# tesseract-robotics/trajopt

Measured on NVIDIA H100. Metric: converged trajectories/sec (7-DOF x 30 wp, batch 1024), higher is better.
Workload: dtype f64

## Files before the change

trajopt_b200/csrc/device_types.cuh:

```cuda
#pragma once
#include <cstdint>

namespace tb200 {

constexpr int kMaxDof = 16;
constexpr int kMaxSeg = 40;
constexpr int kMaxSpheres = 32;
constexpr int kMaxSteps = 64;

struct DevSegment {
  int parent, joint_type, q_index, pad;
  double R[9];
  double p[3];
  double axis[3];
};
struct DevSphere {
  int segment, pad;
  double c[3];
  double r;
};

enum ObjKind {
  OBJ_JOINT_EQ_COST = 0,
  OBJ_JOINT_INEQ_COST = 1,
  OBJ_JOINT_EQ_CNT = 2,
  OBJ_JOINT_INEQ_CNT = 3,
  OBJ_CART_POSE = 4,
  OBJ_COLL = 5,
  OBJ_CART_VEL = 6,
  OBJ_COLL_CAST = 7
};
struct DevObj {
  int kind;
  int is_cnt;
  int order;
  int first;
  int n_steps;
  int term;
  int src_off;
  int n_rows;
  int link;
  int target_slot;
  int pad0;
  int pad1;
  double coeff, margin, buffer;
  double lvs;
};
struct DevJointTerm {
  double coeffs[kMaxDof], targets[kMaxDof], upper[kMaxDof], lower[kMaxDof];
};
struct DevCartTerm {
  double src_R[9], src_p[3];
  double tgt[7];
  int idx[6];
  double coeff[6];
  int n_idx, pad;
};

enum RowInt { RI_BASE = 0, RI_CNT, RI_STRIDE, RI_AUX, RI_OBJ, RI_PAD, RI_NINTS };
enum AuxKind { AUX_NONE = 0, AUX_HINGE = 1, AUX_ABS = 2 };

struct QpSettings {
  double rho, sigma, alpha, eps_abs, eps_rel, eps_prim_inf, eps_dual_inf, delta, adaptive_rho_tolerance;
  int max_iter, scaling, check_termination, adaptive_rho, adaptive_rho_interval, polishing, polish_refine_iter,
      warm_starting, early_polish_every, early_polish_from;
};
struct SqpParams {
  double improve_ratio_threshold, min_trust_box_size, min_approx_improve, min_approx_improve_frac;
  double trust_shrink_ratio, trust_expand_ratio, cnt_tolerance, max_merit_coeff_increases;
  double merit_coeff_increase_ratio, initial_merit_error_coeff, trust_box_size;
  int max_iter, max_qp_solver_failures, inflate_constraints_individually, pad;
};

struct DevProblem {
  int B, T, D, N, HB;
  int S, L, O, obstacles_per_traj;
  int n_costs, n_cnts, n_cart_rows, cart_stride, n_coll_cand, coll_stride;
  int n_cart_targets, n_fixed, max_rows, row_stride, coll_words;
  int n_sparse_lists, n_band;
  int band_offs[32];
  const DevSegment* segs;
  const DevSphere* spheres;
  const double* lower;
  const double* upper;
  const DevObj* cost_objs;
  const DevObj* cnt_objs;
  const DevJointTerm* joint_terms;
  const DevCartTerm* cart_terms;
  const int* fixed_vars;
  const double* Pband;
  const double* qlin;
  const double* init_traj;
  const double* cart_targets;
  const double* obstacles;
  double* x;
  double* new_x;
  double* trust;
  double* merit_coeffs;
  double* cost_vals;
  double* cnt_viols;
  double* new_cost_vals;
  double* new_cnt_viols;
  double* model_cost_vals;
  double* model_cnt_viols;
  int* status;
  int* sqp_iter;
  int* merit_round;
  int* qp_failures;
  int* qp_status;
  int* cur_buf;
  int* n_qp_solves;
  int* n_func_evals;
  int* n_admm_iters;
  int* active_count;
  double* cart_err;
  double* cart_jac;
  double* coll_rows;
  unsigned long long* coll_mask;
  int n_coll_objs, pad2;
  double* rows;
  int* row_ints;
  int* lists;
  size_t list_stride;
  double* ws_x;
  double* ws_yb;
  double* scratch;
  double* soa;
  size_t soa_stride;
  double* factor_g;
  int* lvs_overflow;
  int* qp_done;
  int* ws_meta;
  double* ws_rho;
  double* trace;
  int* trace_len;
  int trace_cap, pad3;
  double* dbg;
  int* sched_state;
  unsigned long long* sched_timers;
  QpSettings qp;
  SqpParams sqp;
};

}
```

trajopt_b200/csrc/kernels.h:

```cpp
#pragma once
#include "device_types.cuh"

namespace tb200 {
struct EvalExtra;
struct SolveCtl;
using SolveKernelFn = void (*)(DevProblem, EvalExtra, SolveCtl);
using EvalKernelFn = void (*)(DevProblem, EvalExtra, int, const double*);
SolveKernelFn solve_kernel_for(int D, bool pair_rows);
EvalKernelFn eval_kernel_for(int D);
int eval_debug_prof(unsigned long long* out, int reset);
int qp_debug_prof(unsigned long long* out, int reset);
}
```

trajopt_b200/csrc/qp_cta_kernel.cuh:

```cuda
#pragma once
#include "device_types.cuh"
#include "joint_terms.cuh"

namespace tb200 {

#ifdef TB200_PROFILE
static __device__ unsigned long long g_prof[16];
#define PROF_T0() const long long prof_t0_ = clock64()
#define PROF_ADD(slot) do { if (q.tid == 0) atomicAdd(&g_prof[slot], (unsigned long long)(clock64() - prof_t0_)); } while (0)
#else
#define PROF_T0()
#define PROF_ADD(slot)
#endif
#if defined(TB200_PROFILE) && defined(TB200_PROFILE_CHECK)
#define PROF_CHK_T0() long long pc_ = clock64()
#define PROF_CHK(slot) do { const long long n_ = clock64(); if (q.tid == 0) atomicAdd(&g_prof[slot], (unsigned long long)(n_ - pc_)); pc_ = n_; } while (0)
#else
#define PROF_CHK_T0()
#define PROF_CHK(slot)
#endif

constexpr int kQpThreads = 256;
constexpr int kQpThreadsC = 256;
constexpr double kOsqpInf = 1e30;
constexpr double kMinScaling = 1e-4, kMaxScaling = 1e4;
constexpr double kVerifyTol = 1e-9;
constexpr int kVerifyRounds = 3;
constexpr double kRhoMin = 1e-6, kRhoMax = 1e6, kRhoTol = 1e-4, kRhoEqOverIneq = 1e3;
enum { QPS_UNSOLVED = 0, QPS_SOLVED = 1, QPS_SOLVED_INACC = 2, QPS_PINF = 3, QPS_PINF_INACC = 4, QPS_DINF = 5,
       QPS_DINF_INACC = 6, QPS_MAXITER = 7, QPS_NONCVX = 8 };

__device__ __forceinline__ double limit_scaling(double v) {
  v = v < kMinScaling ? 1.0 : v;
  return v > kMaxScaling ? kMaxScaling : v;
}

struct QpSmem {
  int SA, SLM, SU, beta, x, zb, yb, v1, w, qs, lbs, ubs, Dz, v2, Pb, tmp, red, colptr, colent, rints, rows, total, row_cap;
  int factor_smem, pband_smem;
  int pinv;
};

struct PinvPlan {
  int ok;
  int Ns, nS;
  int PR;
  int ZS, HO;
  int WS;
  int SS;
  int zo, wo, so;
  int total;
};
__host__ __device__ inline PinvPlan pinv_plan(int M, int nb) {
  PinvPlan pl;
  pl.Ns = M / 4;
  pl.nS = pl.Ns * nb;
  pl.PR = (M - pl.Ns) * nb;
  const int Np = M * nb, blk = nb * nb;
  pl.ok = (nb % 2 == 0) && nb <= 14 && pl.Ns <= 3 && pl.PR + 2 * pl.nS <= 256;
  pl.ZS = Np + ((4 - Np % 16) + 16) % 16;
  pl.HO = ((Np / 2 + 6) / 16) * 16 + 2;
  if (pl.HO > Np) pl.HO = Np;
  pl.WS = 2 * nb + 2;
  pl.SS = pl.nS + (pl.nS & 1);
  const int fA = (M * blk + 15) & ~15, fL = fA + 8, fU = (M * blk + 1) & ~1;
  const int zn = pl.nS * pl.ZS;
  pl.zo = 0;
  pl.wo = ((zn > fA + fL + fU ? zn : fA + fL + fU) + 15) & ~15;
  pl.so = pl.wo + ((pl.PR * pl.WS + 1) & ~1);
  pl.total = pl.so + pl.nS * pl.SS;
  return pl;
}
constexpr int kQpSmemBudget = 28800;
__host__ __device__ inline int qp_block_count(int N, int nb) { return (N + nb - 1) / nb; }
__host__ __device__ inline int qp_even(int v) { return (v + 1) & ~1; }
__host__ __device__ inline int qp_factor_doubles(int N, int nb) { return 3 * qp_even(qp_block_count(N, nb) * nb * nb); }
__host__ __device__ inline size_t qp_cta_global_doubles(int N, int nb) {
  const PinvPlan pl = pinv_plan(qp_block_count(N, nb), nb);
  return static_cast<size_t>(qp_factor_doubles(N, nb)) + static_cast<size_t>(pl.nS) * pl.ZS;
}
__host__ __device__ inline QpSmem qp_smem_layout(int N, int nb, int row_stride, int CN, int max_rows, bool factor_global) {
  const int M = qp_block_count(N, nb), Np = M * nb, blk = nb * nb;
  QpSmem s;
  int o = 0;
  s.beta = o; o += qp_even(Np);
  s.x = o;    o += qp_even(Np);
  s.zb = o;   o += qp_even(Np);
  s.yb = o;   o += qp_even(Np);
  s.v1 = o;   o += qp_even(Np);
  s.w = o;    o += qp_even(Np);
  s.qs = o;   o += qp_even(Np);
  s.lbs = o;  o += qp_even(Np);
  s.ubs = o;  o += qp_even(Np);
  s.Dz = o;   o += qp_even(Np);
  s.v2 = o;   o += qp_even(Np);
  s.tmp = o;  o += 2 * kQpThreadsC + 64 + 8;
  s.red = o;  o += 16 * 8;
  s.colptr = o; o += qp_even((Np + 2) / 2 + 1);
  const int fA = (M * blk + 15) & ~15, fL = fA + 8, fU = qp_even(M * blk);
  s.factor_smem = (!factor_global && o + fA + fL + fU <= kQpSmemBudget) ? 1 : 0;
  o = s.factor_smem ? ((o + 15) & ~15) : o;
  const int per_row2 = 2 * row_stride + CN + RI_NINTS;
  const PinvPlan pl = pinv_plan(M, nb);
  {
    const int region = qp_even(pl.total > fA + fL + fU ? pl.total : fA + fL + fU);
    const int o2 = o + region + qp_even(N * (nb + 1));
    const int cap2 = (o2 < kQpSmemBudget) ? 2 * (kQpSmemBudget - o2) / per_row2 - 1 : 0;
    s.pinv = (s.factor_smem && pl.ok && cap2 >= (max_rows < 64 ? max_rows : 64)) ? 1 : 0;
  }
  s.SA = o;   o += s.factor_smem ? fA : 0;
  s.SLM = o;  o += s.factor_smem ? fL : 0;
  s.SU = o;   o += s.factor_smem ? fU : 0;
  if (s.pinv && s.SA + pl.total > o) o = s.SA + qp_even(pl.total);
  s.pband_smem = (o + qp_even(N * (nb + 1)) <= kQpSmemBudget) ? 1 : 0;
  s.Pb = o;   o += s.pband_smem ? qp_even(N * (nb + 1)) : 0;
  int cap = (o < kQpSmemBudget) ? 2 * (kQpSmemBudget - o) / per_row2 - 1 : 0;
  cap = cap > max_rows ? max_rows : cap;
  cap = cap > 1023 ? 1023 : cap;
  cap = cap < 0 ? 0 : cap;
  s.row_cap = cap;
  s.colent = o; o += qp_even((cap * CN + 1) / 2);
  s.rints = o;  o += qp_even((cap * RI_NINTS + 1) / 2);
  s.rows = o;   o += cap * row_stride;
  s.total = o;
  return s;
}

enum RowF {
  R_C = 0, R_W,
  R_E, R_DA0, R_DA1, R_EA0, R_EA1,
  R_U0, R_U1, R_B0, R_B1, R_LO, R_UP, R_QA0, R_QA1, R_RHO,
  R_XA0, R_XA1, R_Z, R_Y, R_ZA0, R_ZA1, R_YA0, R_YA1,
  R_RA0, R_RA1, R_COEF, R_WR, R_G0, R_G1, R_DEN, R_WRR,
  R_IDEN, R_IWRR,
  R_DY, R_DYA0, R_DYA1, R_DXA0, R_DXA1,
  R_PW, R_PWA0, R_PWA1, R_PB, R_PY, R_PYA0, R_PYA1, R_PX0, R_PX1,
  R_MV,
  R_NF
};
__host__ __device__ inline int qp_row_stride(int CN) { return 3 * CN + R_NF; }

struct SmVec {
  int off;
  __device__ __forceinline__ double* ptr() const {
    extern __shared__ double sm[];
    return sm + off;
  }
  __device__ __forceinline__ double& operator[](int i) const { return ptr()[i]; }
  __device__ __forceinline__ operator double*() const { return ptr(); }
  __device__ __forceinline__ SmVec& operator=(double* p) {
    extern __shared__ double sm[];
    off = static_cast<int>(p - sm);
    return *this;
  }
};

struct QpCtx {
  int N, Np, nb, M, T, D, CN, RS, tid, nrows;
  double *SA, *SLM, *SU;
  SmVec beta, x, zb, yb, v1, w, qs, lbs, ubs, tmp, red, flag;
  int* colptr;
  SmVec Dz, v2;
  double* rows;
  double* soa;
  double* smbase;
// ... 569 lines not shown
      if (mine && R.fu_store) v[R.fu_dst] -= a + o;
    }
    __syncthreads();
  }
  PROF_LVL(15);
  for (int l = R.n_lvl - 1; l >= 1; --l) {
    const bool mine = R.bu_level == l;
    if (__any_sync(0xffffffffu, mine)) {
      double acc = bcr_bwd_task<NB>(sm_base + (mine ? R.bu_X : 0), sm_base + (mine ? R.bu_Um : 0),
                                    (R.bu_yw ? w : v) + (mine ? R.bu_y : 0), w + (mine ? R.bu_wl : 0), R.bu_yw, R.bu_hasl,
                                    R.bu_hasr);
      acc = mine ? acc : 0.0;
      const double o = __shfl_xor_sync(0xffffffffu, acc, 1);
      if (mine && R.bu_store) w[R.bu_dst] = acc + o;
    }
    __syncthreads();
  }
  PROF_LVL(9);
  if (wbase < R.b0_warps) {
    const double acc = bcr_bwd_task<NB>(sm_base + R.b0_X, sm_base + R.b0_Um, (side ? w : v) + R.b0_y, w + R.b0_wl, side,
                                        R.b0_hasl, R.b0_hasr);
    const double o = __shfl_xor_sync(0xffffffffu, acc, 1);
    if (R.b0_store) w[R.b0_dst] = acc + o;
  }
  __syncthreads();
}

template <int NB>
__device__ __forceinline__ double reg_fwd_task(const double (&m)[NB], const double* yv) {
  constexpr int H = NB / 2;
  double2 yy[H];
#pragma unroll
  for (int k = 0; k < H; ++k) yy[k] = lds_v2(yv + 2 * k);
  double a0 = 0.0, a1 = 0.0;
#pragma unroll
  for (int k = 0; k < H; ++k) {
    a0 += m[2 * k] * yy[k].x;
    a1 += m[2 * k + 1] * yy[k].y;
  }
  return a0 + a1;
}
template <int NB>
__device__ __forceinline__ double reg_bwd_task(const double (&m)[NB + NB / 2], const double* y, const double* wl, bool side,
                                               bool hasl, bool hasr) {
  constexpr int H = NB / 2;
  double2 yy[H];
  double ww[H];
#pragma unroll
  for (int k = 0; k < H; ++k) yy[k] = lds_v2(y + 2 * k);
#pragma unroll
  for (int k = 0; k < H; ++k) ww[k] = lds_f64(wl + k);
  double a0 = 0.0, a1 = 0.0, a2 = 0.0;
#pragma unroll
  for (int k = 0; k < H; ++k) {
    a0 += m[2 * k] * yy[k].x;
    a1 += m[2 * k + 1] * yy[k].y;
  }
#pragma unroll
  for (int k = 0; k < H; ++k) a2 += m[NB + k] * ww[k];
  const double dx = a0 + a1;
  return (side ? (hasr ? -dx : 0.0) : dx) - (hasl ? a2 : 0.0);
}
template <int NB>
__device__ __forceinline__ void bcr_solve_regs(const int tid, const SolveRoles& R, const double (&mF0)[NB],
                                               const double (&mB0)[NB + NB / 2], const double (&mFU)[NB],
                                               const double (&mBU)[NB + NB / 2], double* v, double* w) {
  const int wbase = tid & ~31;
  const bool side = tid & 1;
  __syncthreads();
  if (wbase < R.f0_warps) {
    double a = reg_fwd_task<NB>(mF0, v + R.f0_vec);
    a = R.f0_valid ? a : 0.0;
    const double o = __shfl_xor_sync(0xffffffffu, a, 1);
    if (R.f0_store) v[R.f0_dst] -= a + o;
  }
  __syncthreads();
  for (int l = 1; l < R.n_fwd; ++l) {
    const bool mine = R.fu_level == l;
    if (__any_sync(0xffffffffu, mine)) {
      double a = reg_fwd_task<NB>(mFU, v + (mine ? R.fu_vec : 0));
      a = (mine && R.fu_valid) ? a : 0.0;
      const double o = __shfl_xor_sync(0xffffffffu, a, 1);
      if (mine && R.fu_store) v[R.fu_dst] -= a + o;
    }
    __syncthreads();
  }
  for (int l = R.n_lvl - 1; l >= 1; --l) {
    const bool mine = R.bu_level == l;
    if (__any_sync(0xffffffffu, mine)) {
      double acc = reg_bwd_task<NB>(mBU, (R.bu_yw ? w : v) + (mine ? R.bu_y : 0), w + (mine ? R.bu_wl : 0), R.bu_yw,
                                    R.bu_hasl, R.bu_hasr);
      acc = mine ? acc : 0.0;
      const double o = __shfl_xor_sync(0xffffffffu, acc, 1);
      if (mine && R.bu_store) w[R.bu_dst] = acc + o;
    }
    __syncthreads();
  }
  if (wbase < R.b0_warps) {
    const double acc = reg_bwd_task<NB>(mB0, (side ? w : v) + R.b0_y, w + R.b0_wl, side, R.b0_hasl, R.b0_hasr);
    const double o = __shfl_xor_sync(0xffffffffu, acc, 1);
    if (R.b0_store) w[R.b0_dst] = acc + o;
  }
  __syncthreads();
}

template <int NB>
__device__ __forceinline__ void bcr_solve_hyb(const int tid, const SolveRoles& R, const double (&mF0)[NB],
                                              const double (&mB0)[NB + NB / 2], const double* sm_base, double* v, double* w) {
  const int wbase = tid & ~31;
  const bool side = tid & 1;
  __syncthreads();
  if (wbase < R.f0_warps) {
#ifndef TB200_HYB_F0_REGS
    double a = bcr_fwd_task<NB>(sm_base + R.f0_mat, v + R.f0_vec);
#else
    double a = reg_fwd_task<NB>(mF0, v + R.f0_vec);
#endif
    a = R.f0_valid ? a : 0.0;
    const double o = __shfl_xor_sync(0xffffffffu, a, 1);
    if (R.f0_store) v[R.f0_dst] -= a + o;
  }
  __syncthreads();
  for (int l = 1; l < R.n_fwd; ++l) {
    const bool mine = R.fu_level == l;
    if (__any_sync(0xffffffffu, mine)) {
      double a = bcr_fwd_task<NB>(sm_base + (mine ? R.fu_mat : 0), v + (mine ? R.fu_vec : 0));
      a = (mine && R.fu_valid) ? a : 0.0;
      const double o = __shfl_xor_sync(0xffffffffu, a, 1);
      if (mine && R.fu_store) v[R.fu_dst] -= a + o;
    }
    __syncthreads();
  }
  for (int l = R.n_lvl - 1; l >= 1; --l) {
    const bool mine = R.bu_level == l;
    if (__any_sync(0xffffffffu, mine)) {
      double acc = bcr_bwd_task<NB>(sm_base + (mine ? R.bu_X : 0), sm_base + (mine ? R.bu_Um : 0),
                                    (R.bu_yw ? w : v) + (mine ? R.bu_y : 0), w + (mine ? R.bu_wl : 0), R.bu_yw, R.bu_hasl,
                                    R.bu_hasr);
      acc = mine ? acc : 0.0;
      const double o = __shfl_xor_sync(0xffffffffu, acc, 1);
      if (mine && R.bu_store) w[R.bu_dst] = acc + o;
    }
    __syncthreads();
  }
  if (wbase < R.b0_warps) {
    const double acc = reg_bwd_task<NB>(mB0, (side ? w : v) + R.b0_y, w + R.b0_wl, side, R.b0_hasl, R.b0_hasr);
    const double o = __shfl_xor_sync(0xffffffffu, acc, 1);
    if (R.b0_store) w[R.b0_dst] = acc + o;
  }
  __syncthreads();
}

template <int NB>
__device__ __forceinline__ void p_matvec(const QpCtx& q, const double* in, double* out) {
  extern __shared__ double sm[];
  constexpr int HB = NB, W = HB + 1;
  const int N = q.N, Np = q.Np, nbo = q.n_band;
  const double* const Pb = q.Pband;
  const double* const Dz = sm + (q.Dz - q.smbase);
  const double* const vin = sm + (in - q.smbase);
  double* const vout = sm + (out - q.smbase);
  const int* const offs = q.band_offs;
  const double cc = q.c;
  for (int i = q.tid; i < Np; i += kQpThreads) {
    double s = 0.0;
    if (i < N) {
      for (int t0 = 0; t0 < nbo; t0 += 4) {
        double v[4];
#pragma unroll
        for (int u = 0; u < 4; ++u) {
          const int k = (t0 + u < nbo) ? offs[t0 + u] : -1;
          v[u] = (k >= 0 && k <= i) ? (Pb[i * W + k] * Dz[i - k]) * vin[i - k] : 0.0;
        }
        s += v[0]; s += v[1]; s += v[2]; s += v[3];
      }
      for (int t0 = 0; t0 < nbo; t0 += 4) {
        double v[4];
#pragma unroll
        for (int u = 0; u < 4; ++u) {
          const int k = (t0 + u < nbo) ? offs[t0 + u] : -1;
          v[u] = (k >= 1 && i + k < N) ? (Pb[(i + k) * W + k] * Dz[i + k]) * vin[i + k] : 0.0;
        }
        s += v[0]; s += v[1]; s += v[2]; s += v[3];
      }
      s *= cc * Dz[i];
    }
    vout[i] = s;
  }
  __syncthreads();
}

__device__ inline void rows_prepare_weights(const QpCtx& q, const SysW& w) {
  for (int r = q.tid; r < q.nrows; r += kQpThreads) {
    double* F = q.F(r);
    const int naux = q.I(r)[RI_AUX];
    const double Wr = w.polish ? fabs(F[R_PW]) : ((F[R_RHO] != 0.0) ? q.rho_eq : q.rho);
    const double wa0 = w.polish ? fabs(F[R_PWA0]) : w.rho_aux;
    const double wa1 = w.polish ? fabs(F[R_PWA1]) : w.rho_aux;
    const double g0 = (naux >= 1) ? w.sig + wa0 * F[R_B0] * F[R_B0] : 1.0;
    const double g1 = (naux == 2) ? w.sig + wa1 * F[R_B1] * F[R_B1] : 1.0;
    const double den = g0 * g1 + Wr * (F[R_U0] * F[R_U0] * g1 + F[R_U1] * F[R_U1] * g0);
    F[R_WRR] = Wr;
    F[R_G0] = g0;
    F[R_G1] = g1;
    F[R_DEN] = den;
    F[R_IDEN] = 1.0 / den;
    F[R_IWRR] = (Wr != 0.0) ? 1.0 / Wr : 0.0;
    F[R_WR] = Wr * g0 * g1 / den;
  }
  __syncthreads();
}
__device__ __forceinline__ double xbound_weight(const QpCtx& q, const SysW& w, int j) {
  const double adm = (q.ubs[j] - q.lbs[j] < kRhoTol) ? q.rho_eq : q.rho;
  return w.polish ? fabs(q.zb[j]) : adm;
}

__device__ __forceinline__ double pivot_rcp(const double x) {
  double r;
  asm("rcp.approx.ftz.f64 %0, %1;" : "=d"(r) : "d"(x));
  double e = fma(-x, r, 1.0);
  r = fma(r, e, r);
  e = fma(-x, r, 1.0);
  r = fma(r, e, r);
  e = fma(-x, r, 1.0);
  return fma(r, e, r);
}
template <int QN>
__device__ __forceinline__ bool gj_rows(double (&a)[QN], double diag, const bool active, const int mat, const int row,
                                        const int n, const int n_max, double* tmp, const int nmat) {
  constexpr int BS = QN + 2;
  double* const csv = tmp + 2 * nmat * BS + mat * QN;
  bool bad = false;
  double pv_mine = pivot_rcp(diag), my_cs = 1.0, rs = 1.0, inv_rs = 1.0;
#pragma unroll 1
  for (int k = 0; k < n_max; ++k) {
    double* buf = tmp + ((k & 1) * nmat + mat) * BS;
    const bool piv = active && row == k;
    if (piv) {
      bad |= !(diag > 0.0);
#pragma unroll
      for (int j = 0; j < QN; j += 2) *reinterpret_cast<double2*>(buf + j) = make_double2(a[j], a[j + 1]);
      buf[k] = 0.0;
      buf[QN] = pv_mine;
      my_cs = -pv_mine;
      csv[k] = my_cs;
      rs = pv_mine;
      inv_rs = diag;
      diag = pv_mine;
    }
    __syncthreads();
    if (active && k < n && !piv) {
      const double tr = buf[row];
      const bool ahead = row > k;
      const double f = ahead ? tr : -tr * my_cs;
      const double g = f * buf[QN];
      diag = ahead ? diag - g * f : diag + g * f;
      const double gs = g * inv_rs;
#pragma unroll
      for (int j = 0; j < QN; j += 2) {
        const double2 t = *reinterpret_cast<const double2*>(buf + j);
        a[j] -= gs * t.x;
        a[j + 1] -= gs * t.y;
      }
      if (ahead) pv_mine = pivot_rcp(diag);
    }
  }
  if (active) {
#pragma unroll
    for (int j = 0; j < QN; ++j) a[j] = (j == row) ? diag : ((j < n) ? a[j] * (rs * csv[j]) : 0.0);
  }
  return bad;
}

template <int NB>
__device__ inline bool pinv_factor(const QpCtx& q) {
  constexpr int QN = 3 * NB, blk = NB * NB;
  static_assert(QN % 2 == 0, "pivot rows move as double2");
  extern __shared__ double sm[];
  const int tid = q.tid, M = q.M, Np = q.Np;
  const int PR = q.pl.PR, nS = q.pl.nS, Ns = q.pl.Ns, ZS = q.pl.ZS, WS = q.pl.WS, SS = q.pl.SS;
  double* const fbase = sm + (q.SA - q.smbase);
  const double* const SA = fbase;
  const double* const SLM = sm + (q.SLM - q.smbase);
  double* const Z = fbase + q.pl.zo;
  double* const W = fbase + q.pl.wo;
  double* const S = fbase + q.pl.so;
  double* const tmp = q.tmp.ptr();
  const int nparts = (M + 3) / 4;
  bool bad = false;
#ifdef TB200_PROFILE
  long long pf_ = clock64();
#define PROF_PF(slot) do { const long long n_ = clock64(); if (tid == 0) atomicAdd(&g_prof[slot], (unsigned long long)(n_ - pf_)); pf_ = n_; } while (0)
#else
#define PROF_PF(slot)
#endif
  {
    const bool prow = tid < PR;
    const int p = prow ? tid / QN : 0, lr = prow ? tid % QN : 0;
    const int npb = (M - 4 * p) < 3 ? (M - 4 * p) : 3;
    const int kb = lr / NB, r = lr % NB, gb = 4 * p + kb;
    double a[QN];
#pragma unroll
    for (int j = 0; j < QN; ++j) {
      const int cb = j / NB, c = j % NB;
      double v = 0.0;
      if (prow && cb < npb) {
        if (cb == kb) v = SA[gb * blk + r * NB + c];
        else if (cb == kb - 1) v = SLM[gb * blk + r * NB + c];
        else if (cb == kb + 1) v = SLM[(gb + 1) * blk + c * NB + r];
      }
      a[j] = v;
    }
    PROF_PF(0);
    const double dg = prow ? SA[gb * blk + r * NB + r] : 1.0;
    bad |= gj_rows<QN>(a, dg, prow, p, lr, npb * NB, (M < 3 ? M : 3) * NB, tmp, nparts);
    PROF_PF(4);
    if (prow) {
#pragma unroll
      for (int j = 0; j < QN; ++j) q.pi_g[tid * QN + j] = a[j];
      const bool has_l = p > 0, has_r = 4 * p + 3 < M;
#pragma unroll 2
      for (int j = 0; j < NB; ++j) {
        double wl = 0.0, wr = 0.0;
        if (has_l) {
#pragma unroll
          for (int c = 0; c < NB; ++c) wl += a[c] * SLM[(4 * p) * blk + c * NB + j];
        }
        if (has_r) {
#pragma unroll
          for (int c = 0; c < NB; ++c) wr += a[2 * NB + c] * SLM[(4 * p + 3) * blk + j * NB + c];
        }
        W[tid * WS + j] = wl;
        W[tid * WS + NB + j] = wr;
      }
    }
  }
  __syncthreads();
  for (int e = tid; e < nS * nS; e += kQpThreads) {
    const int ra = e / nS, ca = e % nS, sa = ra / NB, i = ra % NB, sb = ca / NB, j = ca % NB;
    double v = 0.0;
    if (sa == sb || sb == sa + 1 || sb == sa - 1) {
      const bool use_l = sb <= sa, use_r = sb >= sa && 4 * sa + 4 < M;
      const double* cl = SLM + (4 * sa + 3) * blk + i * NB;
// ... 329 lines not shown
  double* const v1 = sm + (q.v1 - q.smbase);
  double* const w = sm + (q.w - q.smbase);
  double* const rows = sm + (q.rows - q.smbase);
  const int* const rints = reinterpret_cast<const int*>(sm + (reinterpret_cast<const double*>(q.rints) - q.smbase));
  const int* const colent = reinterpret_cast<const int*>(sm + (reinterpret_cast<const double*>(q.colent) - q.smbase));
  double* const dxs = q.scratch;
  double* const dyb = q.scratch + Np;
  const SolveRoles roles = solve_roles<NB>(q);
  double mF0[NB], mB0[NB + NB / 2];
  load_fwd_row<NB>(q, 0, tid, mF0);
  load_bwd_row<NB>(q, 0, tid, mB0);
  const bool has_var = tid < N;
  const int vi = has_var ? tid : 0;
  const double v_beta = q.beta[vi], v_lb = q.lbs[vi], v_ub = q.ubs[vi], v_qs = q.qs[vi];
  const bool v_eq = v_ub - v_lb < kRhoTol;
  const double v_rb = v_eq ? rho_eq : rho, v_irb = v_eq ? inv_rho_eq : inv_rho;
  double v_x = q.x[vi], v_z = q.zb[vi], v_y = q.yb[vi];
  const int e0 = has_var ? q.colptr[vi] : 0, e1 = has_var ? q.colptr[vi + 1] : 0;
  double* const zero_slot = sm + (q.flag - q.smbase) + 7;
  if (tid == 0) *zero_slot = 0.0;
  int ea[kPre];
#pragma unroll
  for (int k = 0; k < kPre; ++k) {
    const int e = e0 + k;
    const int ent = (e < e1) ? colent[e] : -1;
    ea[k] = (ent >= 0) ? static_cast<int>(rows - sm) + (ent >> 5) * RS + (2 * CNc + R_NF) + (ent & 31)
                       : static_cast<int>(zero_slot - sm);
  }
  {
    PROF_T0();
    for (int r = kQpThreads - 1 - tid; r < nrows; r += kQpThreads) {
      double* F = rows + r * RS + 2 * CNc;
      const double s = F[R_WRR] * F[R_Z] - F[R_Y];
      const double ra0 = sigma * F[R_XA0] - F[R_QA0] + F[R_U0] * s + F[R_B0] * (rho_aux * F[R_ZA0] - F[R_YA0]);
      const double ra1 = sigma * F[R_XA1] - F[R_QA1] + F[R_U1] * s + F[R_B1] * (rho_aux * F[R_ZA1] - F[R_YA1]);
      F[R_RA0] = ra0;
      F[R_RA1] = ra1;
      const double cf = row_reduce_coef(F, ra0, ra1, s);
      F[R_COEF] = cf;
      const double* as = rows + r * RS + CNc;
#pragma unroll
      for (int k = 0; k < CNc; ++k) F[R_NF + k] = as[k] * cf;
    }
    __syncthreads();
    PROF_ADD(0);
  }
  for (int it = 0; it < n_iter; ++it) {
    const bool keep_steps = keep_last && it == n_iter - 1;
    {
      PROF_T0();
      double s = 0.0;
      if (has_var) {
        s = sigma * v_x - v_qs + v_beta * (v_rb * v_z - v_y);
        double c[kPre];
#pragma unroll
        for (int k = 0; k < kPre; ++k) c[k] = sm[ea[k]];
        if constexpr (kPre == 8) s += ((c[0] + c[1]) + (c[2] + c[3])) + ((c[4] + c[5]) + (c[6] + c[7]));
        else s += (c[0] + c[1]) + (c[2] + c[3]);
        for (int e = e0 + kPre; e < e1; ++e) {
          const int ent = colent[e];
          s += rows[(ent >> 5) * RS + (2 * CNc + R_NF) + (ent & 31)];
        }
      }
      if (tid < Np) v1[tid] = s;
      PROF_ADD(1);
    }
    {
      PROF_T0();
      bcr_solve_hyb<NB>(tid, roles, mF0, mB0, sm, v1, w);
      PROF_ADD(2);
    }
    PROF_T0();
    for (int r = kQpThreads - 1 - tid; r < nrows; r += kQpThreads) {
      const double* R = rows + r * RS;
      double* F = rows + r * RS + 2 * CNc;
      const int* I = rints + r * RI_NINTS;
      double zeta = 0.0;
      {
        const int base = I[RI_BASE], stride = I[RI_STRIDE], last = I[RI_CNT] - 1;
#pragma unroll
        for (int k = 0; k < CNc; ++k) zeta += R[CNc + k] * w[base + min(k, last) * stride];
      }
      double a0, a1;
      row_backsub(F, zeta, a0, a1);
      const double zt = zeta + F[R_U0] * a0 + F[R_U1] * a1;
      const double Wr = F[R_WRR];
      const double zr = alpha * zt + oma * F[R_Z];
      double zn = zr + F[R_Y] * F[R_IWRR];
      zn = fmin(fmax(zn, F[R_LO]), F[R_UP]);
      const double dy = Wr * (zr - zn);
      const double yn = F[R_Y] + dy;
      F[R_Z] = zn;
      F[R_Y] = yn;
      F[R_DY] = dy;
      const double s = Wr * zn - yn;
      double ra[2];
#pragma unroll
      for (int k = 0; k < 2; ++k) {
        const double at = k ? a1 : a0, bb = F[R_B0 + k];
        const double xo = F[R_XA0 + k];
        const double xn = alpha * at + oma * xo;
        const double zra = alpha * (bb * at) + oma * F[R_ZA0 + k];
        double z2 = zra + F[R_YA0 + k] * inv_rho_aux;
        z2 = fmin(fmax(z2, 0.0), kOsqpInf * F[R_EA0 + k]);
        const double dya = rho_aux * (zra - z2);
        const double yan = F[R_YA0 + k] + dya;
        F[R_XA0 + k] = xn;
        F[R_DXA0 + k] = xn - xo;
        F[R_ZA0 + k] = z2;
        F[R_YA0 + k] = yan;
        F[R_DYA0 + k] = dya;
        ra[k] = sigma * xn - F[R_QA0 + k] + F[R_U0 + k] * s + bb * (rho_aux * z2 - yan);
      }
      F[R_RA0] = ra[0];
      F[R_RA1] = ra[1];
      const double cf = row_reduce_coef(F, ra[0], ra[1], s);
      F[R_COEF] = cf;
#pragma unroll
      for (int k = 0; k < CNc; ++k) F[R_NF + k] = R[CNc + k] * cf;
    }
    if (has_var) {
      const double xt = w[vi];
      const double xn = alpha * xt + oma * v_x;
      const double zr = alpha * (v_beta * xt) + oma * v_z;
      double zn = zr + v_y * v_irb;
      zn = fmin(fmax(zn, v_lb), v_ub);
      const double dy = v_rb * (zr - zn);
      if (keep_steps) {
        dxs[vi] = xn - v_x;
        dyb[vi] = dy;
      }
      v_x = xn;
      v_z = zn;
      v_y += dy;
    }
    __syncthreads();
    PROF_ADD(3);
  }
  if (has_var) {
    q.x[vi] = v_x;
    q.zb[vi] = v_z;
    q.yb[vi] = v_y;
  }
  __syncthreads();
}

template <int NB, int PAIR>
__device__ __noinline__ void admm_block_pinv(const QpCtx& q, const double rho_aux_in, const int n_iter, const int keep_last) {
  constexpr int CNc = PAIR ? ((NB > 3) ? NB : 3) : ((NB / 2 > 3) ? NB / 2 : 3);
  constexpr int kPre = 8;
  constexpr int QN = 3 * NB;
  constexpr int kRowThreads = 64;
  extern __shared__ double sm[];
  const int tid = q.tid, N = q.N, Np = q.Np, nrows = q.nrows, RS = q.RS;
  const double sigma = q.sigma, alpha = q.alpha, oma = 1.0 - q.alpha, rho = q.rho, rho_eq = q.rho_eq, rho_aux = rho_aux_in;
  const double inv_rho_aux = 1.0 / rho_aux, inv_rho = 1.0 / rho, inv_rho_eq = 1.0 / rho_eq;
  double* const v1 = sm + (q.v1 - q.smbase);
  double* const w = sm + (q.w - q.smbase);
  double* const rows = sm + (q.rows - q.smbase);
  const int* const rints = reinterpret_cast<const int*>(sm + (reinterpret_cast<const double*>(q.rints) - q.smbase));
  const int* const colent = reinterpret_cast<const int*>(sm + (reinterpret_cast<const double*>(q.colent) - q.smbase));
  double* const dxs = q.scratch;
  double* const dyb = q.scratch + Np;
  const int M = q.M, PR = q.pl.PR, nS = q.pl.nS, ZS = q.pl.ZS, HO = q.pl.HO, WS = q.pl.WS;
  const double* const fbase = sm + (q.SA - q.smbase);
  const bool upper = tid >= kQpThreads - kRowThreads;
  const bool prow = tid < PR;
  const int pp = prow ? tid / QN : 0, plr = prow ? tid % QN : 0;
  const int pb0 = pp * 4 * NB, pvar = pb0 + plr;
  const int pn = ((M - 4 * pp) < 3 ? (M - 4 * pp) : 3) * NB;
  const int xl_off = (pp > 0) ? (4 * pp - 1) * NB : 0;
  const int xr_off = (4 * pp + 3 < M) ? (4 * pp + 3) * NB : 0;
  const unsigned a_wrow = smem_u32(fbase + q.pl.wo + (prow ? tid : 0) * WS);
  const unsigned a_b = smem_u32(v1 + pb0), a_xl = smem_u32(w + xl_off), a_xr = smem_u32(w + xr_off);
  const bool swork = tid >= PR && tid < PR + 2 * nS;
  const int sw = swork ? tid - PR : 0, srow = sw >> 1, half = sw & 1;
  const int svar = (4 * (srow / NB) + 3) * NB + srow % NB;
  const int c0 = half ? HO : 0, c1 = half ? Np : HO;
  const unsigned a_z = smem_u32(fbase + q.pl.zo + srow * ZS), a_v1 = smem_u32(v1);
  const bool has_var = tid < N;
  const int vi = has_var ? tid : 0;
  const double v_beta = q.beta[vi], v_lb = q.lbs[vi], v_ub = q.ubs[vi], v_qs = q.qs[vi];
  const bool v_eq = v_ub - v_lb < kRhoTol;
  const double v_rb = v_eq ? rho_eq : rho, v_irb = v_eq ? inv_rho_eq : inv_rho;
  double v_x = q.x[vi], v_z = q.zb[vi], v_y = q.yb[vi];
  const int e0 = has_var ? q.colptr[vi] : 0, e1 = has_var ? q.colptr[vi + 1] : 0;
  double* const zero_slot = sm + (q.flag - q.smbase) + 7;
  if (tid == 0) *zero_slot = 0.0;
  int ea[kPre];
#pragma unroll
  for (int k = 0; k < kPre; ++k) {
    const int e = e0 + k;
    const int ent = (e < e1) ? colent[e] : -1;
    ea[k] = (ent >= 0) ? static_cast<int>(rows - sm) + (ent >> 5) * RS + (2 * CNc + R_NF) + (ent & 31)
                       : static_cast<int>(zero_slot - sm);
  }
  auto bar = []() { asm volatile("bar.sync 0;" ::: "memory"); };
  auto build_rhs = [&]() {
    double s = 0.0;
    if (has_var) {
      s = sigma * v_x - v_qs + v_beta * (v_rb * v_z - v_y);
      double c[kPre];
#pragma unroll
      for (int k = 0; k < kPre; ++k) c[k] = sm[ea[k]];
      s += ((c[0] + c[1]) + (c[2] + c[3])) + ((c[4] + c[5]) + (c[6] + c[7]));
      for (int e = e0 + kPre; e < e1; ++e) {
        const int ent = colent[e];
        s += rows[(ent >> 5) * RS + (2 * CNc + R_NF) + (ent & 31)];
      }
    }
    if (tid < Np) v1[tid] = s;
  };
  auto sep_half = [&]() {
    double zs = 0.0;
    if (swork) {
      double s0 = 0.0, s1 = 0.0, s2 = 0.0, s3 = 0.0;
      int c = c0;
      unsigned az = a_z + c0 * 8, ab = a_v1 + c0 * 8;
#pragma unroll 2
      for (; c + 8 <= c1; c += 8, az += 64, ab += 64) {
        const double2 z0 = lds_v2_at(az), z1 = lds_v2_at(az + 16), z2 = lds_v2_at(az + 32), z3 = lds_v2_at(az + 48);
        const double2 b0 = lds_v2_at(ab), b1 = lds_v2_at(ab + 16), b2 = lds_v2_at(ab + 32), b3 = lds_v2_at(ab + 48);
        s0 += z0.x * b0.x; s1 += z0.y * b0.y; s2 += z1.x * b1.x; s3 += z1.y * b1.y;
        s0 += z2.x * b2.x; s1 += z2.y * b2.y; s2 += z3.x * b3.x; s3 += z3.y * b3.y;
      }
      for (; c < c1; c += 2, az += 16, ab += 16) {
        const double2 z0 = lds_v2_at(az), b0 = lds_v2_at(ab);
        s0 += z0.x * b0.x; s1 += z0.y * b0.y;
      }
      zs = (s0 + s1) + (s2 + s3);
    }
    zs += __shfl_xor_sync(0xffffffffu, zs, 1);
    if (swork && half == 0) w[svar] = zs;
  };
  auto var_update = [&](const bool keep_steps) {
    if (has_var) {
      const double xt = w[vi];
      const double xn = alpha * xt + oma * v_x;
      const double zr = alpha * (v_beta * xt) + oma * v_z;
      double zn = zr + v_y * v_irb;
      zn = fmin(fmax(zn, v_lb), v_ub);
      const double dy = v_rb * (zr - zn);
      if (keep_steps) {
        dxs[vi] = xn - v_x;
        dyb[vi] = dy;
      }
      v_x = xn;
      v_z = zn;
      v_y += dy;
    }
  };

  if (!upper) {
    double pi[QN];
#pragma unroll
    for (int j = 0; j < QN; ++j) pi[j] = prow ? q.pi_g[tid * QN + j] : 0.0;
    bar();
    for (int it = 0; it < n_iter; ++it) {
      const bool keep_steps = keep_last && it == n_iter - 1;
      { PROF_T0(); build_rhs(); PROF_ADD(1); }
      {
        PROF_T0();
        PROF_CHK_T0();
        bar();
        PROF_CHK(4);
        double y = 0.0;
        if (prow) {
          double y0 = 0.0, y1 = 0.0;
#pragma unroll
          for (int j = 0; j < QN; j += 2) {
            double2 bb = make_double2(0.0, 0.0);
            if (j < pn) bb = lds_v2_at(a_b + j * 8);
            y0 += pi[j] * bb.x;
            y1 += pi[j + 1] * bb.y;
          }
          y = y0 + y1;
        }
        sep_half();
        PROF_CHK(14);
        bar();
        PROF_CHK(15);
        if (prow) {
          double t0 = 0.0, t1 = 0.0;
#pragma unroll
          for (int t = 0; t < NB; t += 2) {
            const double2 wl = lds_v2_at(a_wrow + t * 8), wr = lds_v2_at(a_wrow + (NB + t) * 8);
            const double2 xl = lds_v2_at(a_xl + t * 8), xr = lds_v2_at(a_xr + t * 8);
            t0 += wl.x * xl.x + wr.x * xr.x;
            t1 += wl.y * xl.y + wr.y * xr.y;
          }
          w[pvar] = y - (t0 + t1);
        }
        bar();
        PROF_CHK(9);
        PROF_ADD(2);
      }
      {
        PROF_T0();
        var_update(keep_steps);
        bar();
        PROF_ADD(3);
      }
    }
  } else {
    for (int r = kQpThreads - 1 - tid; r < nrows; r += kRowThreads) {
      double* F = rows + r * RS + 2 * CNc;
      const double s = F[R_WRR] * F[R_Z] - F[R_Y];
      const double ra0 = sigma * F[R_XA0] - F[R_QA0] + F[R_U0] * s + F[R_B0] * (rho_aux * F[R_ZA0] - F[R_YA0]);
      const double ra1 = sigma * F[R_XA1] - F[R_QA1] + F[R_U1] * s + F[R_B1] * (rho_aux * F[R_ZA1] - F[R_YA1]);
      F[R_RA0] = ra0;
      F[R_RA1] = ra1;
      const double cf = row_reduce_coef(F, ra0, ra1, s);
      F[R_COEF] = cf;
      const double* as = rows + r * RS + CNc;
#pragma unroll
      for (int k = 0; k < CNc; ++k) F[R_NF + k] = as[k] * cf;
    }
    bar();
    for (int it = 0; it < n_iter; ++it) {
      const bool keep_steps = keep_last && it == n_iter - 1;
      build_rhs();
      bar();
      sep_half();
      bar();
      bar();
      for (int r = kQpThreads - 1 - tid; r < nrows; r += kRowThreads) {
        const double* R = rows + r * RS;
        double* F = rows + r * RS + 2 * CNc;
        const int* I = rints + r * RI_NINTS;
        double zeta = 0.0;
        {
          const int base = I[RI_BASE], stride = I[RI_STRIDE], last = I[RI_CNT] - 1;
#pragma unroll
          for (int k = 0; k < CNc; ++k) zeta += R[CNc + k] * w[base + min(k, last) * stride];
        }
        double a0, a1;
        row_backsub(F, zeta, a0, a1);
        const double zt = zeta + F[R_U0] * a0 + F[R_U1] * a1;
        const double Wr = F[R_WRR];
        const double zr = alpha * zt + oma * F[R_Z];
        double zn = zr + F[R_Y] * F[R_IWRR];
        zn = fmin(fmax(zn, F[R_LO]), F[R_UP]);
        const double dy = Wr * (zr - zn);
        const double yn = F[R_Y] + dy;
        F[R_Z] = zn;
        F[R_Y] = yn;
        F[R_DY] = dy;
        const double s = Wr * zn - yn;
        double ra[2];
#pragma unroll
        for (int k = 0; k < 2; ++k) {
          const double at = k ? a1 : a0, bb = F[R_B0 + k];
          const double xo = F[R_XA0 + k];
          const double xn = alpha * at + oma * xo;
          const double zra = alpha * (bb * at) + oma * F[R_ZA0 + k];
          double z2 = zra + F[R_YA0 + k] * inv_rho_aux;
          z2 = fmin(fmax(z2, 0.0), kOsqpInf * F[R_EA0 + k]);
          const double dya = rho_aux * (zra - z2);
          const double yan = F[R_YA0 + k] + dya;
          F[R_XA0 + k] = xn;
          F[R_DXA0 + k] = xn - xo;
          F[R_ZA0 + k] = z2;
          F[R_YA0 + k] = yan;
          F[R_DYA0 + k] = dya;
          ra[k] = sigma * xn - F[R_QA0 + k] + F[R_U0 + k] * s + bb * (rho_aux * z2 - yan);
        }
        F[R_RA0] = ra[0];
        F[R_RA1] = ra[1];
        const double cf = row_reduce_coef(F, ra[0], ra[1], s);
        F[R_COEF] = cf;
#pragma unroll
        for (int k = 0; k < CNc; ++k) F[R_NF + k] = R[CNc + k] * cf;
      }
      var_update(keep_steps);
      bar();
    }
  }
  if (has_var) {
    q.x[vi] = v_x;
    q.zb[vi] = v_z;
    q.yb[vi] = v_y;
  }
  __syncthreads();
}

enum SoaF { S_U0 = 0, S_U1, S_B0, S_B1, S_LO, S_UP, S_QA0, S_QA1, S_WRR, S_IWRR, S_G0, S_G1, S_IDEN, S_UPA0, S_UPA1,
            S_Z, S_Y, S_XA0, S_XA1, S_ZA0, S_ZA1, S_YA0, S_YA1, S_RA0, S_RA1, S_AS };
__host__ __device__ inline size_t qp_soa_doubles(int max_rows, int CN) {
  const size_t rsd = (static_cast<size_t>(max_rows) + 31) & ~static_cast<size_t>(31);
  return rsd * (S_AS + CN) + (rsd * (3 + CN) + 1) / 2 + static_cast<size_t>(max_rows) * CN + 8;
}
template <int NB, int PAIR>
__device__ __noinline__ void admm_block_soa(const QpCtx& q, const double rho_aux_in, const int n_iter, const int keep_last) {
  constexpr int CNc = PAIR ? ((NB > 3) ? NB : 3) : ((NB / 2 > 3) ? NB / 2 : 3);
  const int N = q.N, Np = q.Np, tid = q.tid, nrows = q.nrows;
  const double sigma = q.sigma, alpha = q.alpha, oma = 1.0 - q.alpha, rho = q.rho, rho_eq = q.rho_eq, rho_aux = rho_aux_in;
  const double inv_rho_aux = 1.0 / rho_aux, inv_rho = 1.0 / rho, inv_rho_eq = 1.0 / rho_eq;
  double* const dxs = q.scratch;
  double* const dyb = q.scratch + Np;
  const int RSd = (nrows + 31) & ~31;
  double* const sd = q.soa;
  int* const si = reinterpret_cast<int*>(sd + static_cast<size_t>(RSd) * (S_AS + CNc));
  double* const ct = sd + static_cast<size_t>(RSd) * (S_AS + CNc) + (static_cast<size_t>(RSd) * (3 + CNc) + 1) / 2 + 1;
  const int nnz = q.colptr[Np];
  PROF_T0();
  for (int i = tid; i < N; i += kQpThreads)
    for (int e = q.colptr[i]; e < q.colptr[i + 1]; ++e) {
      const int ent = q.colent[e];
      si[(3 + (ent & 31)) * RSd + (ent >> 5)] = e;
    }
  for (int e = tid; e < nnz; e += kQpThreads) ct[e] = 0.0;
  __syncthreads();
  for (int r = tid; r < nrows; r += kQpThreads) {
    const double* R = q.R(r);
    const double* F = q.F(r);
    const int* I = q.I(r);
    const int cnt = I[RI_CNT];
    si[r] = I[RI_BASE];
    si[RSd + r] = I[RI_STRIDE];
    si[2 * RSd + r] = cnt - 1;
    sd[S_U0 * RSd + r] = F[R_U0]; sd[S_U1 * RSd + r] = F[R_U1]; sd[S_B0 * RSd + r] = F[R_B0]; sd[S_B1 * RSd + r] = F[R_B1];
    sd[S_LO * RSd + r] = F[R_LO]; sd[S_UP * RSd + r] = F[R_UP]; sd[S_QA0 * RSd + r] = F[R_QA0]; sd[S_QA1 * RSd + r] = F[R_QA1];
    sd[S_WRR * RSd + r] = F[R_WRR]; sd[S_IWRR * RSd + r] = F[R_IWRR]; sd[S_G0 * RSd + r] = F[R_G0]; sd[S_G1 * RSd + r] = F[R_G1];
    sd[S_IDEN * RSd + r] = F[R_IDEN];
    sd[S_UPA0 * RSd + r] = kOsqpInf * F[R_EA0]; sd[S_UPA1 * RSd + r] = kOsqpInf * F[R_EA1];
    sd[S_Z * RSd + r] = F[R_Z]; sd[S_Y * RSd + r] = F[R_Y]; sd[S_XA0 * RSd + r] = F[R_XA0]; sd[S_XA1 * RSd + r] = F[R_XA1];
    sd[S_ZA0 * RSd + r] = F[R_ZA0]; sd[S_ZA1 * RSd + r] = F[R_ZA1]; sd[S_YA0 * RSd + r] = F[R_YA0]; sd[S_YA1 * RSd + r] = F[R_YA1];
    const double s0 = F[R_WRR] * F[R_Z] - F[R_Y];
    const double ra0 = sigma * F[R_XA0] - F[R_QA0] + F[R_U0] * s0 + F[R_B0] * (rho_aux * F[R_ZA0] - F[R_YA0]);
    const double ra1 = sigma * F[R_XA1] - F[R_QA1] + F[R_U1] * s0 + F[R_B1] * (rho_aux * F[R_ZA1] - F[R_YA1]);
    sd[S_RA0 * RSd + r] = ra0;
    sd[S_RA1 * RSd + r] = ra1;
    const double cf = row_reduce_coef(F, ra0, ra1, s0);
#pragma unroll
    for (int k = 0; k < CNc; ++k) {
      const double a = R[CNc + k];
      sd[(S_AS + k) * RSd + r] = a;
      if (k < cnt) ct[si[(3 + k) * RSd + r]] = a * cf;
    }
  }
  __syncthreads();
  PROF_ADD(0);
  for (int it = 0; it < n_iter; ++it) {
    const bool keep_steps = keep_last && it == n_iter - 1;
    long long pt_ = 0;
#ifdef TB200_PROFILE
    pt_ = clock64();
#define PROF_SOA(slot) do { const long long n_ = clock64(); if (tid == 0) atomicAdd(&g_prof[slot], (unsigned long long)(n_ - pt_)); pt_ = n_; } while (0)
#else
#define PROF_SOA(slot) (void)pt_
#endif
    for (int i = tid; i < Np; i += kQpThreads) {
      double s = 0.0;
      if (i < N) {
        const double rb = (q.ubs[i] - q.lbs[i] < kRhoTol) ? rho_eq : rho;
        s = sigma * q.x[i] - q.qs[i] + q.beta[i] * (rb * q.zb[i] - q.yb[i]);
        const int e1 = q.colptr[i + 1];
        for (int e = q.colptr[i]; e < e1; ++e) s += ct[e];
      }
      q.v1[i] = s;
    }
    PROF_SOA(1);
    bcr_solve<NB>(q, q.v1, q.w);
    PROF_SOA(2);
    for (int r = tid; r < nrows; r += kQpThreads) {
      const int base = si[r], stride = si[RSd + r], last = si[2 * RSd + r];
      double as[CNc];
#pragma unroll
      for (int k = 0; k < CNc; ++k) as[k] = sd[(S_AS + k) * RSd + r];
      const double U0 = sd[S_U0 * RSd + r], U1 = sd[S_U1 * RSd + r], B0 = sd[S_B0 * RSd + r], B1 = sd[S_B1 * RSd + r];
      const double LO = sd[S_LO * RSd + r], UP = sd[S_UP * RSd + r], QA0 = sd[S_QA0 * RSd + r], QA1 = sd[S_QA1 * RSd + r];
      const double Wr = sd[S_WRR * RSd + r], IWRR = sd[S_IWRR * RSd + r], G0 = sd[S_G0 * RSd + r], G1 = sd[S_G1 * RSd + r];
      const double iden = sd[S_IDEN * RSd + r], UPA0 = sd[S_UPA0 * RSd + r], UPA1 = sd[S_UPA1 * RSd + r];
      const double Z = sd[S_Z * RSd + r], Y = sd[S_Y * RSd + r], XA0 = sd[S_XA0 * RSd + r], XA1 = sd[S_XA1 * RSd + r];
      const double ZA0 = sd[S_ZA0 * RSd + r], ZA1 = sd[S_ZA1 * RSd + r], YA0 = sd[S_YA0 * RSd + r], YA1 = sd[S_YA1 * RSd + r];
      const double ra0o = sd[S_RA0 * RSd + r], ra1o = sd[S_RA1 * RSd + r];
      double zeta = 0.0;
#pragma unroll
      for (int k = 0; k < CNc; ++k) zeta += as[k] * q.w[base + min(k, last) * stride];
      const double a0 = (G1 * (ra0o - Wr * U0 * zeta) + Wr * U1 * (U1 * ra0o - U0 * ra1o)) * iden;
      const double a1 = (G0 * (ra1o - Wr * U1 * zeta) + Wr * U0 * (U0 * ra1o - U1 * ra0o)) * iden;
      const double zt = zeta + U0 * a0 + U1 * a1;
      const double zr = alpha * zt + oma * Z;
      double zn = zr + Y * IWRR;
      zn = fmin(fmax(zn, LO), UP);
      const double dy = Wr * (zr - zn);
      const double yn = Y + dy;
      const double s = Wr * zn - yn;
      const double xn0 = alpha * a0 + oma * XA0;
      const double zra0 = alpha * (B0 * a0) + oma * ZA0;
      double z20 = zra0 + YA0 * inv_rho_aux;
      z20 = fmin(fmax(z20, 0.0), UPA0);
      const double dya0 = rho_aux * (zra0 - z20);
      const double yan0 = YA0 + dya0;
      const double ra0 = sigma * xn0 - QA0 + U0 * s + B0 * (rho_aux * z20 - yan0);
      const double xn1 = alpha * a1 + oma * XA1;
      const double zra1 = alpha * (B1 * a1) + oma * ZA1;
      double z21 = zra1 + YA1 * inv_rho_aux;
      z21 = fmin(fmax(z21, 0.0), UPA1);
      const double dya1 = rho_aux * (zra1 - z21);
      const double yan1 = YA1 + dya1;
      const double ra1 = sigma * xn1 - QA1 + U1 * s + B1 * (rho_aux * z21 - yan1);
      const double cf = s - Wr * (U0 * ra0 * G1 + U1 * ra1 * G0) * iden;
      sd[S_Z * RSd + r] = zn; sd[S_Y * RSd + r] = yn; sd[S_XA0 * RSd + r] = xn0; sd[S_XA1 * RSd + r] = xn1;
      sd[S_ZA0 * RSd + r] = z20; sd[S_ZA1 * RSd + r] = z21; sd[S_YA0 * RSd + r] = yan0; sd[S_YA1 * RSd + r] = yan1;
      sd[S_RA0 * RSd + r] = ra0; sd[S_RA1 * RSd + r] = ra1;
#pragma unroll
      for (int k = 0; k < CNc; ++k)
        if (k <= last) ct[si[(3 + k) * RSd + r]] = as[k] * cf;
      if (it == n_iter - 1) {
        double* F = q.F(r);
        F[R_Z] = zn; F[R_Y] = yn; F[R_DY] = dy;
        F[R_XA0] = xn0; F[R_XA1] = xn1; F[R_DXA0] = xn0 - XA0; F[R_DXA1] = xn1 - XA1;
        F[R_ZA0] = z20; F[R_ZA1] = z21; F[R_YA0] = yan0; F[R_YA1] = yan1; F[R_DYA0] = dya0; F[R_DYA1] = dya1;
        F[R_RA0] = ra0; F[R_RA1] = ra1; F[R_COEF] = cf;
      }
    }
    for (int i = tid; i < N; i += kQpThreads) {
      const double beta = q.beta[i];
      const double lb = q.lbs[i], ub = q.ubs[i];
      const bool beq = ub - lb < kRhoTol;
      const double rb = beq ? rho_eq : rho, irb = beq ? inv_rho_eq : inv_rho;
      const double xt = q.w[i];
      const double xn = alpha * xt + oma * q.x[i];
      const double zr = alpha * (beta * xt) + oma * q.zb[i];
      double zn = zr + q.yb[i] * irb;
      zn = fmin(fmax(zn, lb), ub);
      const double dy = rb * (zr - zn);
      if (keep_steps) {
        dxs[i] = xn - q.x[i];
        dyb[i] = dy;
      }
      q.x[i] = xn;
      q.zb[i] = zn;
      q.yb[i] += dy;
    }
    __syncthreads();
    PROF_SOA(3);
  }
}

__device__ inline void qp_scale(QpCtx& q, const QpSettings& st, int n_aux_total) {
  double *qs = q.qs, *lbs = q.lbs, *ubs = q.ubs;
  const int N = q.N, tid = q.tid, HB = 2 * q.D, W = HB + 1;
  double* Eb = q.zb;
  q.c = 1.0;
  for (int i = tid; i < q.Np; i += kQpThreads) {
    q.Dz[i] = 1.0;
    Eb[i] = 1.0;
  }
  for (int r = tid; r < q.nrows; r += kQpThreads) {
    double* F = q.F(r);
    F[R_E] = F[R_DA0] = F[R_DA1] = F[R_EA0] = F[R_EA1] = 1.0;
  }
  __syncthreads();
  for (int pass = 0; pass < st.scaling; ++pass) {
    for (int r = tid; r < q.nrows; r += kQpThreads) {
      double* R = q.R(r);
      double* F = q.F(r);
      const int* I = q.I(r);
      const int base = I[RI_BASE], cnt = I[RI_CNT], stride = I[RI_STRIDE], aux = I[RI_AUX];
      const double E = F[R_E];
      double rn = 0.0;
      for (int k = 0; k < cnt; ++k) rn = fmax(rn, fabs(E * R[k] * q.Dz[base + k * stride]));
      double dt0 = 1.0, dt1 = 1.0, et0 = 1.0, et1 = 1.0;
      if (aux >= 1) {
        const double ua = fabs(E * F[R_DA0]), ba = fabs(F[R_EA0] * F[R_DA0]);
        rn = fmax(rn, ua);
        dt0 = 1.0 / sqrt(limit_scaling(fmax(ua, ba)));
        et0 = 1.0 / sqrt(limit_scaling(ba));
      }
      if (aux == 2) {
        const double ua = fabs(E * F[R_DA1]), ba = fabs(F[R_EA1] * F[R_DA1]);
        rn = fmax(rn, ua);
        dt1 = 1.0 / sqrt(limit_scaling(fmax(ua, ba)));
        et1 = 1.0 / sqrt(limit_scaling(ba));
      }
      F[R_RA0] = 1.0 / sqrt(limit_scaling(rn));
      F[R_RA1] = E;
      F[R_DA0] *= dt0;
      F[R_DA1] *= dt1;
      F[R_EA0] *= et0;
      F[R_EA1] *= et1;
    }
    __syncthreads();
    for (int i = tid; i < N; i += kQpThreads) {
      double m = 0.0;
      for (int t = 0; t < q.n_band; ++t) {
        const int k = q.band_offs[t];
        if (k <= i) m = fmax(m, fabs(q.c * q.Dz[i] * q.Pband[i * W + k] * q.Dz[i - k]));
        if (k >= 1 && i + k < N) m = fmax(m, fabs(q.c * q.Dz[i] * q.Pband[(i + k) * W + k] * q.Dz[i + k]));
      }
      const double bn = fabs(Eb[i] * q.Dz[i]);
      m = fmax(m, bn);
      for (int e = q.colptr[i]; e < q.colptr[i + 1]; ++e) {
        const int ent = q.colent[e], r = ent >> 5, k = ent & 31;
        const double* R = q.R(r);
        m = fmax(m, fabs(R[2 * q.CN + R_RA1] * R[k] * q.Dz[i]));
      }
      q.v1[i] = 1.0 / sqrt(limit_scaling(m));
      Eb[i] *= 1.0 / sqrt(limit_scaling(bn));
    }
    __syncthreads();
    for (int i = tid; i < N; i += kQpThreads) q.Dz[i] *= q.v1[i];
    for (int r = tid; r < q.nrows; r += kQpThreads) {
      double* F = q.F(r);
      F[R_E] = F[R_RA1] * F[R_RA0];
    }
    __syncthreads();
    double csum = 0.0, qn = 0.0;
    for (int i = tid; i < N; i += kQpThreads) {
      double m = 0.0;
      for (int t = 0; t < q.n_band; ++t) {
        const int k = q.band_offs[t];
        if (k <= i) m = fmax(m, fabs(q.c * q.Dz[i] * q.Pband[i * W + k] * q.Dz[i - k]));
        if (k >= 1 && i + k < N) m = fmax(m, fabs(q.c * q.Dz[i] * q.Pband[(i + k) * W + k] * q.Dz[i + k]));
      }
      csum += m;
      qn = fmax(qn, fabs(q.c * q.Dz[i] * qs[i]));
    }
    for (int r = tid; r < q.nrows; r += kQpThreads) {
      const double* F = q.F(r);
      const int aux = q.I(r)[RI_AUX];
      if (aux >= 1) qn = fmax(qn, fabs(q.c * F[R_DA0] * F[R_W]));
      if (aux == 2) qn = fmax(qn, fabs(q.c * F[R_DA1] * F[R_W]));
    }
    double red2[2] = {csum, qn};
    block_reduce<2, 0x1u>(q, red2);
    const double mean = limit_scaling(red2[0] / static_cast<double>(N + n_aux_total));
    q.c *= 1.0 / fmax(mean, limit_scaling(red2[1]));
  }
  q.cinv = 1.0 / q.c;
  for (int i = tid; i < q.Np; i += kQpThreads) {
    if (i < N) {
      qs[i] = q.c * q.Dz[i] * qs[i];
      lbs[i] *= Eb[i];
      ubs[i] *= Eb[i];
      q.beta[i] = Eb[i] * q.Dz[i];
    } else {
      qs[i] = 0.0; lbs[i] = -1.0; ubs[i] = 1.0; q.beta[i] = 1.0; q.Dz[i] = 1.0;
    }
  }
  for (int r = tid; r < q.nrows; r += kQpThreads) {
    double* R = q.R(r);
    double* F = q.F(r);
    const int* I = q.I(r);
    const int aux = I[RI_AUX];
    const double E = F[R_E];
    for (int k = 0; k < q.CN; ++k) R[q.CN + k] = E * R[k] * q.Dz[row_var(I, k)];
    F[R_U0] = F[R_U1] = F[R_B0] = F[R_B1] = F[R_QA0] = F[R_QA1] = 0.0;
    F[R_UP] = -F[R_C] * E;
    if (aux == AUX_HINGE) {
      F[R_U0] = -E * F[R_DA0];
      F[R_B0] = F[R_EA0] * F[R_DA0];
      F[R_QA0] = q.c * F[R_DA0] * F[R_W];
      F[R_LO] = -kOsqpInf * E;
      F[R_RHO] = 0.0;
    } else {
      if (aux == AUX_ABS) {
        F[R_U0] = E * F[R_DA0];
        F[R_U1] = -E * F[R_DA1];
        F[R_B0] = F[R_EA0] * F[R_DA0];
        F[R_B1] = F[R_EA1] * F[R_DA1];
        F[R_QA0] = q.c * F[R_DA0] * F[R_W];
        F[R_QA1] = q.c * F[R_DA1] * F[R_W];
      }
      F[R_LO] = F[R_UP];
      F[R_RHO] = 1.0;
    }
  }
  __syncthreads();
}

template <int NB, int PAIR, bool REGOK>
__device__ inline QpOut qp_solve_block(QpCtx& q, const QpSettings& st, bool warm, double warm_rho,
                                       const double* ws_x, const double* ws_yb) {
  constexpr int CNc = PAIR ? ((NB > 3) ? NB : 3) : ((NB / 2 > 3) ? NB / 2 : 3);
  const int N = q.N, tid = q.tid;
  QpOut out{QPS_UNSOLVED, 0, 0, st.rho, 0, 0, 0, 0, 0, -1, 0, 0};
  double rho;
  double eps_scale;
  int iter, round;
  q.sigma = st.sigma;
  q.alpha = st.alpha;
  {
    rho = warm ? warm_rho : st.rho;
    rho = fmin(fmax(rho, kRhoMin), kRhoMax);
    eps_scale = 1.0;
    iter = 0;
    round = 0;
    q.rho = rho;
    q.rho_eq = kRhoEqOverIneq * rho;
    if (warm) {
      for (int i = tid; i < q.Np; i += kQpThreads) {
        if (i < N) {
          q.x[i] = ws_x[i] / q.Dz[i];
          q.yb[i] = ws_yb[i] * q.Dz[i] / q.beta[i] * q.c;
          q.zb[i] = q.beta[i] * q.x[i];
        } else {
          q.x[i] = q.yb[i] = q.zb[i] = 0.0;
        }
      }
      __syncthreads();
      for (int r = tid; r < q.nrows; r += kQpThreads) {
        double* R = q.R(r);
        double* F = q.F(r);
        const int naux = q.I(r)[RI_AUX];
        F[R_XA0] = (naux >= 1) ? F[R_XA0] / F[R_DA0] : 0.0;
        F[R_XA1] = (naux == 2) ? F[R_XA1] / F[R_DA1] : 0.0;
        F[R_Y] = F[R_Y] / F[R_E] * q.c;
        F[R_YA0] = (naux >= 1) ? F[R_YA0] / F[R_EA0] * q.c : 0.0;
        F[R_YA1] = (naux == 2) ? F[R_YA1] / F[R_EA1] * q.c : 0.0;
        F[R_Z] = row_dot<CNc>(q, R, q.I(r), q.x) + F[R_U0] * F[R_XA0] + F[R_U1] * F[R_XA1];
        F[R_ZA0] = F[R_B0] * F[R_XA0];
        F[R_ZA1] = F[R_B1] * F[R_XA1];
      }
    } else {
      for (int i = tid; i < q.Np; i += kQpThreads) q.x[i] = q.zb[i] = q.yb[i] = 0.0;
      for (int r = tid; r < q.nrows; r += kQpThreads) {
        double* F = q.F(r);
        F[R_XA0] = F[R_XA1] = F[R_Z] = F[R_Y] = F[R_ZA0] = F[R_ZA1] = F[R_YA0] = F[R_YA1] = 0.0;
      }
    }
    __syncthreads();
  }
  SysW sysw{false, st.sigma, rho};
  bool factor_ok = true;

  const bool use_reg = REGOK && solve_roles_fit(q.M, NB);
  const bool use_pinv = REGOK && q.pinv && q.rows_smem;
  using BlockFn = void (*)(const QpCtx&, double, int, int);
  auto run_block = [&](int n, bool keep_last) {
    if constexpr (REGOK) {
      if (use_pinv || use_reg) {
        BlockFn volatile fn = use_pinv ? &admm_block_pinv<NB, PAIR>
                                       : (q.rows_smem ? &admm_block_fast<NB, PAIR> : &admm_block_soa<NB, PAIR>);
        fn(q, sysw.rho_aux, n, keep_last ? 1 : 0);
        return;
      }
    }
    BlockFn volatile fn = q.rows_smem ? &admm_block<NB, PAIR, false> : &admm_block_soa<NB, PAIR>;
    fn(q, sysw.rho_aux, n, keep_last ? 1 : 0);
  };
  using FactorFn = bool (*)(const QpCtx&, const SysW&);
  auto factorize = [&](const SysW& wts) -> bool {
    if constexpr (REGOK) {
      if (use_pinv && !wts.polish) {
        FactorFn volatile fn = &assemble_factor<NB, true>;
        return fn(q, wts);
      }
    }
    FactorFn volatile fn = &assemble_factor<NB, false>;
    return fn(q, wts);
  };
  auto stash_z = [&](const bool restore) {
    extern __shared__ double sm[];
    double2* zs = reinterpret_cast<double2*>(sm + (q.SA - q.smbase) + q.pl.zo);
    double2* zg = reinterpret_cast<double2*>(q.z_stash);
    const int n2 = q.pl.nS * q.pl.ZS / 2;
    if (restore) for (int i = tid; i < n2; i += kQpThreads) zs[i] = zg[i];
    else for (int i = tid; i < n2; i += kQpThreads) zg[i] = zs[i];
    __syncthreads();
    if (restore) rows_prepare_weights(q, sysw);
  };
  { PROF_T0(); factor_ok = factorize(sysw); PROF_ADD(6); }

  double* dxs = q.scratch;
  double* dyb = q.scratch + q.Np;
  double* st_x = q.scratch + 2 * q.Np;
  double* st_zb = q.scratch + 3 * q.Np;
  double* st_yb = q.scratch + 4 * q.Np;
  double pri_res = 0.0, dua_res = 0.0;
  int status = factor_ok ? QPS_UNSOLVED : QPS_NONCVX;
  bool early_verified = false;
  unsigned long long prev_guess = 0ull, failed_guess = 0ull, pending_guess = 0ull;
  bool have_prev_guess = false, have_failed_guess = false;
  double n_z = 0, n_ax = 0, n_q = 0, n_aty = 0, n_px = 0, s_pri = 0, s_dua = 0, s_z = 0, s_ax = 0, s_q = 0, s_aty = 0, s_px = 0;

  auto info_pass = [&](const bool scaled) {
    PROF_CHK_T0();
    p_matvec<NB>(q, q.x, q.v2);
    PROF_CHK(4);
    double m[14] = {0, 0, 0, 0, 0, 0, 0, 0, 0, 0, 0, 0, 0, 0};
    for (int r = tid; r < q.nrows; r += kQpThreads) {
      const double* R = q.R(r);
      double* F = q.F(r);
      const double ax = row_dot<CNc>(q, R, q.I(r), q.x) + F[R_U0] * F[R_XA0] + F[R_U1] * F[R_XA1];
      const double einv = 1.0 / F[R_E];
      m[0] = fmax(m[0], fabs(einv * (ax - F[R_Z])));
      m[1] = fmax(m[1], fabs(einv * F[R_Z]));
      m[2] = fmax(m[2], fabs(einv * ax));
      m[7] = fmax(m[7], fabs(ax - F[R_Z]));
      m[8] = fmax(m[8], fabs(F[R_Z]));
      m[9] = fmax(m[9], fabs(ax));
#pragma unroll
      for (int k = 0; k < 2; ++k) {
        const double u = F[R_U0 + k], bb = F[R_B0 + k], qa = F[R_QA0 + k];
        const double xa = F[R_XA0 + k], za = F[R_ZA0 + k], ya = F[R_YA0 + k];
        const double iea = 1.0 / F[R_EA0 + k], ida = 1.0 / F[R_DA0 + k];
        const double axb = bb * xa;
        m[0] = fmax(m[0], fabs(iea * (axb - za)));
        m[1] = fmax(m[1], fabs(iea * za));
        m[2] = fmax(m[2], fabs(iea * axb));
        m[7] = fmax(m[7], fabs(axb - za));
        m[8] = fmax(m[8], fabs(za));
        m[9] = fmax(m[9], fabs(axb));
        const double aty = u * F[R_Y] + bb * ya;
        m[3] = fmax(m[3], fabs(ida * (qa + aty)));
        m[4] = fmax(m[4], fabs(ida * aty));
        m[5] = fmax(m[5], fabs(ida * qa));
        m[10] = fmax(m[10], fabs(qa + aty));
        m[11] = fmax(m[11], fabs(aty));
        m[12] = fmax(m[12], fabs(qa));
      }
      F[R_COEF] = F[R_Y];
    }
    __syncthreads();
    PROF_CHK(14);
    scatter_columns<CNc>(q, [&](int i) { return q.beta[i] * q.yb[i]; });
    for (int i = tid; i < N; i += kQpThreads) {
      const double dz = q.Dz[i], beta = q.beta[i];
      const double ax = beta * q.x[i], aty = q.v1[i], px = q.v2[i];
      const double einv = dz / beta, dinv = 1.0 / dz;
      m[0] = fmax(m[0], fabs(einv * (ax - q.zb[i])));
      m[1] = fmax(m[1], fabs(einv * q.zb[i]));
      m[2] = fmax(m[2], fabs(einv * ax));
      m[7] = fmax(m[7], fabs(ax - q.zb[i]));
      m[8] = fmax(m[8], fabs(q.zb[i]));
      m[9] = fmax(m[9], fabs(ax));
      const double qv = q.qs[i], d = qv + px + aty;
      m[3] = fmax(m[3], fabs(dinv * d));
      m[4] = fmax(m[4], fabs(dinv * aty));
      m[5] = fmax(m[5], fabs(dinv * qv));
      m[6] = fmax(m[6], fabs(dinv * px));
      m[10] = fmax(m[10], fabs(d));
      m[11] = fmax(m[11], fabs(aty));
      m[12] = fmax(m[12], fabs(qv));
      m[13] = fmax(m[13], fabs(px));
    }
    if (scaled) {
      block_reduce<14, 0u>(q, m);
      s_pri = m[7]; s_z = m[8]; s_ax = m[9]; s_dua = m[10]; s_aty = m[11]; s_q = m[12]; s_px = m[13];
    } else {
      double m7[7] = {m[0], m[1], m[2], m[3], m[4], m[5], m[6]};
      block_reduce<7, 0u>(q, m7);
#pragma unroll
      for (int k = 0; k < 7; ++k) m[k] = m7[k];
    }
    PROF_CHK(15);
    pri_res = m[0];
    dua_res = m[3] * q.cinv;
    n_z = m[1]; n_ax = m[2]; n_aty = m[4]; n_q = m[5]; n_px = m[6];
  };

  auto primal_infeasible = [&](double eps) -> bool {
    double a[3] = {0.0, 0.0, 0.0};
    for (int r = tid; r < q.nrows; r += kQpThreads) {
      double* F = q.F(r);
      const int naux = q.I(r)[RI_AUX];
      double d = F[R_DY];
      d = (naux == AUX_HINGE) ? fmax(d, 0.0) : d;
      a[0] = fmax(a[0], fabs(F[R_E] * d));
      a[1] += F[R_UP] * fmax(d, 0.0) + F[R_LO] * fmin(d, 0.0);
      F[R_COEF] = d;
#pragma unroll
      for (int k = 0; k < 2; ++k) {
        const double da = fmin(F[R_DYA0 + k], 0.0);
        a[0] = fmax(a[0], fabs(F[R_EA0 + k] * da));
        a[2] = fmax(a[2], fabs((F[R_U0 + k] * d + F[R_B0 + k] * da) / F[R_DA0 + k]));
      }
    }
    for (int i = tid; i < N; i += kQpThreads) {
      const double d = dyb[i];
      a[0] = fmax(a[0], fabs(q.beta[i] / q.Dz[i] * d));
      a[1] += q.ubs[i] * fmax(d, 0.0) + q.lbs[i] * fmin(d, 0.0);
    }
    block_reduce<3, 0x2u>(q, a);
    if (!((a[0] > eps) && (a[1] < -eps * a[0]))) return false;
    scatter_columns<CNc>(q, [&](int i) { return q.beta[i] * dyb[i]; });
    double mm[1] = {a[2]};
    for (int i = tid; i < N; i += kQpThreads) mm[0] = fmax(mm[0], fabs(q.v1[i] / q.Dz[i]));
    block_reduce<1, 0u>(q, mm);
    return (a[0] > eps) && (a[1] < -eps * a[0]) && (mm[0] < eps * a[0]);
  };
  auto dual_infeasible = [&](double eps) -> bool {
    double a[2] = {0.0, 0.0};
    for (int i = tid; i < q.Np; i += kQpThreads) {
      const double dxi = (i < N) ? dxs[i] : 0.0;
      if (i < N) {
        a[0] = fmax(a[0], fabs(q.Dz[i] * dxi));
        a[1] += q.qs[i] * dxi;
      }
      q.v1[i] = dxi;
    }
    for (int r = tid; r < q.nrows; r += kQpThreads) {
      const double* F = q.F(r);
#pragma unroll
      for (int k = 0; k < 2; ++k) {
        a[0] = fmax(a[0], fabs(F[R_DA0 + k] * F[R_DXA0 + k]));
        a[1] += F[R_QA0 + k] * F[R_DXA0 + k];
      }
    }
    block_reduce<2, 0x2u>(q, a);
    const double ndx = a[0], qdx = a[1];
    if (!((ndx > eps) && (qdx < -q.c * eps * ndx))) return false;
    p_matvec<NB>(q, q.v1, q.v2);
    double b2[2] = {0.0, 0.0};
    for (int i = tid; i < N; i += kQpThreads) {
      b2[0] = fmax(b2[0], fabs(q.v2[i] / q.Dz[i]));
      const double vv = q.Dz[i] * q.v1[i];
      b2[1] += (vv > eps * ndx || vv < -eps * ndx) ? 1.0 : 0.0;
    }
    for (int r = tid; r < q.nrows; r += kQpThreads) {
      const double* R = q.R(r);
      const double* F = q.F(r);
      const int naux = q.I(r)[RI_AUX];
      const double ax = row_dot<CNc>(q, R, q.I(r), q.v1) + F[R_U0] * F[R_DXA0] + F[R_U1] * F[R_DXA1];
      const double vv = ax / F[R_E];
      b2[1] += (vv > eps * ndx) ? 1.0 : 0.0;
      b2[1] += (naux != AUX_HINGE && vv < -eps * ndx) ? 1.0 : 0.0;
#pragma unroll
      for (int k = 0; k < 2; ++k) {
        const double va = F[R_B0 + k] * F[R_DXA0 + k] / F[R_EA0 + k];
        b2[1] += (k < naux && va < -eps * ndx) ? 1.0 : 0.0;
      }
    }
    block_reduce<2, 0x2u>(q, b2);
    return (ndx > eps) && (qdx < -q.c * eps * ndx) && (b2[0] < q.c * eps * ndx) && (b2[1] == 0.0);
  };
  auto check_termination = [&](bool approximate) -> int {
    double eps_abs = st.eps_abs * eps_scale, eps_rel = st.eps_rel * eps_scale, epi = st.eps_prim_inf, edi = st.eps_dual_inf;
    if (approximate) {
      eps_abs *= 10; eps_rel *= 10; epi *= 10; edi *= 10;
    }
    const double eps_pri = eps_abs + eps_rel * fmax(n_z, n_ax);
    const double eps_dua = eps_abs + eps_rel * q.cinv * fmax(n_q, fmax(n_aty, n_px));
    const bool pri_ok = pri_res < eps_pri, dua_ok = dua_res < eps_dua;
    int res = QPS_UNSOLVED;
    if (pri_res > kOsqpInf || dua_res > kOsqpInf) res = QPS_NONCVX;
    else if (pri_ok && dua_ok) res = approximate ? QPS_SOLVED_INACC : QPS_SOLVED;
    else {
      const bool pinf = pri_ok ? false : primal_infeasible(epi);
      const bool dinf = dua_ok ? false : dual_infeasible(edi);
      if (pinf) res = approximate ? QPS_PINF_INACC : QPS_PINF;
      else if (dinf) res = approximate ? QPS_DINF_INACC : QPS_DINF;
    }
    return res;
  };

  auto guess_mix = [](unsigned long long v) -> unsigned long long {
    v += 0x9e3779b97f4a7c15ull;
    v = (v ^ (v >> 30)) * 0xbf58476d1ce4e5b9ull;
    v = (v ^ (v >> 27)) * 0x94d049bb133111ebull;
    return v ^ (v >> 31);
  };
  auto early_guess_settled = [&]() -> bool {
    unsigned long long h = 0ull;
    const unsigned long long mc = static_cast<unsigned long long>(q.nrows);
    for (int r = tid; r < q.nrows; r += kQpThreads) {
      const double* F = q.F(r);
      const int* I = q.I(r);
      if (F[R_Z] - F[R_LO] < -F[R_Y]) h += guess_mix(2ull * r);
      else if (F[R_UP] - F[R_Z] < F[R_Y]) h += guess_mix(2ull * r + 1ull);
      for (int k = 0; k < I[RI_AUX]; ++k) {
        const unsigned long long idx = mc + N + I[RI_PAD] + k;
        if (F[R_ZA0 + k] - 0.0 < -F[R_YA0 + k]) h += guess_mix(2ull * idx);
        else if (kOsqpInf * F[R_EA0 + k] - F[R_ZA0 + k] < F[R_YA0 + k]) h += guess_mix(2ull * idx + 1ull);
      }
    }
    for (int i = tid; i < N; i += kQpThreads) {
      const unsigned long long idx = mc + i;
      if (q.zb[i] - q.lbs[i] < -q.yb[i]) h += guess_mix(2ull * idx);
      else if (q.ubs[i] - q.zb[i] < q.yb[i]) h += guess_mix(2ull * idx + 1ull);
    }
    __syncwarp();
    for (int off = 16; off > 0; off >>= 1) h += __shfl_xor_sync(0xffffffffu, h, off);
    unsigned long long* red = reinterpret_cast<unsigned long long*>(q.red.ptr());
    if ((tid & 31) == 0) red[tid >> 5] = h;
    __syncthreads();
    h = 0ull;
    for (int w = 0; w < kQpThreads / 32; ++w) h += red[w];
    __syncthreads();
    const bool stable = have_prev_guess && h == prev_guess;
    prev_guess = h;
    have_prev_guess = true;
    pending_guess = h;
    return stable && !(have_failed_guess && h == failed_guess);
  };

  auto run_admm = [&](auto& polish_fn, auto& restore_fn) {
    status = QPS_UNSOLVED;
    bool stop = false;
    while (!stop) {
      if (iter >= st.max_iter) {
        if (!(st.check_termination > 0 && (iter % st.check_termination == 0))) info_pass(false);
        status = check_termination(true);
        if (status == QPS_UNSOLVED) status = QPS_MAXITER;
        stop = true;
      } else {
        int n = st.max_iter - iter;
        if (st.check_termination > 0) n = min(n, st.check_termination - iter % st.check_termination);
        if (st.adaptive_rho && st.adaptive_rho_interval > 0) n = min(n, st.adaptive_rho_interval - iter % st.adaptive_rho_interval);
        iter += n;
        const bool can_check = st.check_termination > 0 && (iter % st.check_termination == 0);
        const bool rho_iter = st.adaptive_rho && st.adaptive_rho_interval > 0 && (iter % st.adaptive_rho_interval == 0);
        run_block(n, can_check || iter == st.max_iter);
        if (can_check) {
          PROF_T0();
          info_pass(rho_iter);
          PROF_CHK_T0();
          status = check_termination(false);
          PROF_CHK(9);
          PROF_ADD(5);
          if (status != QPS_UNSOLVED) stop = true;
          else if (st.polishing && st.early_polish_every > 0 && iter >= st.early_polish_from &&
                   (iter % st.early_polish_every == 0) && early_guess_settled()) {
            bool verified = false;
            double p_pri = 0.0, p_dua = 0.0;
            if (use_pinv) stash_z(false);
            const bool factored = polish_fn(verified, p_pri, p_dua);
            if (factored && verified) {
              early_verified = true;
              out.pol_factor_ok = 1;
              out.pol_pri = p_pri;
              out.pol_dua = p_dua;
              status = QPS_SOLVED;
              stop = true;
            } else {
              failed_guess = pending_guess;
              have_failed_guess = true;
              restore_fn(false);
              info_pass(rho_iter);
              if (use_pinv) {
                stash_z(true);
              } else if (!factorize(sysw)) {
                status = QPS_NONCVX;
                stop = true;
              }
            }
          }
        }
        if (!stop && rho_iter) {
          if (!can_check) info_pass(true);
          const double pn = s_pri / (fmax(s_z, s_ax) + 1e-10);
          const double dn = s_dua / (fmax(s_q, fmax(s_aty, s_px)) + 1e-10);
          double rho_new = rho * sqrt(pn / (dn + 1e-10));
          rho_new = fmin(fmax(rho_new, kRhoMin), kRhoMax);
          if (rho_new > rho * st.adaptive_rho_tolerance || rho_new < rho / st.adaptive_rho_tolerance) {
            rho = rho_new;
            q.rho = rho;
            q.rho_eq = kRhoEqOverIneq * rho;
            sysw.rho_aux = rho;
            out.rho_updates++;
            if (!factorize(sysw)) {
              status = QPS_NONCVX;
              stop = true;
            }
          }
        }
      }
    }
  };

  const double wp = 1.0 / st.delta;
  const SysW pw{true, st.delta, 0.0};
  auto polish_once = [&](bool& verified, double& p_pri, double& p_dua) -> bool {
    PROF_T0();
    verified = false;
    for (int i = tid; i < q.Np; i += kQpThreads) {
      const double z = q.zb[i], y = q.yb[i];
      double w = 0.0;
      if (i < N) {
        if (z - q.lbs[i] < -y) w = -wp;
        else if (q.ubs[i] - z < y) w = wp;
      }
      st_x[i] = q.x[i];
      st_zb[i] = z;
      st_yb[i] = y;
      q.zb[i] = w;
      q.x[i] = 0.0;
      q.yb[i] = 0.0;
    }
    for (int r = tid; r < q.nrows; r += kQpThreads) {
      double* F = q.F(r);
      const int naux = q.I(r)[RI_AUX];
      double w = 0.0, b = 0.0;
      if (F[R_Z] - F[R_LO] < -F[R_Y]) { w = -wp; b = F[R_LO]; }
      else if (F[R_UP] - F[R_Z] < F[R_Y]) { w = wp; b = F[R_UP]; }
      F[R_PW] = w;
      F[R_PB] = b;
      F[R_PY] = 0.0;
#pragma unroll
      for (int k = 0; k < 2; ++k) {
        double wa = 0.0;
        if (k < naux) {
          if (F[R_ZA0 + k] - 0.0 < -F[R_YA0 + k]) wa = -wp;
          else if (kOsqpInf * F[R_EA0 + k] - F[R_ZA0 + k] < F[R_YA0 + k]) wa = wp;
        }
        F[R_PWA0 + k] = wa;
        F[R_PYA0 + k] = 0.0;
        F[R_PX0 + k] = 0.0;
      }
    }
    __syncthreads();
    if (!factorize(pw)) return false;
    for (int it = 0; it <= st.polish_refine_iter + 1; ++it) {
      const bool last = (it == st.polish_refine_iter + 1);
      p_matvec<NB>(q, q.x, q.v2);
      double mm[3] = {0.0, 0.0, 0.0};
      for (int r = tid; r < q.nrows; r += kQpThreads) {
        const double* R = q.R(r);
        double* F = q.F(r);
        const int naux = q.I(r)[RI_AUX];
        const double Wr = F[R_WRR];
        const double ax = row_dot<CNc>(q, R, q.I(r), q.x) + F[R_U0] * F[R_PX0] + F[R_U1] * F[R_PX1];
        const double py = F[R_PY] + ((it > 0) ? Wr * (ax - F[R_PB]) : 0.0);
        const double e = py + (last ? 0.0 : Wr * (ax - F[R_PB]));
        const double zc = fmin(fmax(ax, F[R_LO]), F[R_UP]);
        mm[0] = fmax(mm[0], fabs((ax - zc) / F[R_E]));
        mm[2] += (last && Wr != 0.0 && naux == AUX_HINGE && py < -kVerifyTol) ? 1.0 : 0.0;
        double pya[2], ra[2];
#pragma unroll
        for (int k = 0; k < 2; ++k) {
          const double bb = F[R_B0 + k], u = F[R_U0 + k], qa = F[R_QA0 + k];
          const double wa = fabs(F[R_PWA0 + k]);
          const double axb = bb * F[R_PX0 + k];
          pya[k] = F[R_PYA0 + k] + ((it > 0) ? wa * axb : 0.0);
          const double ea = pya[k] + (last ? 0.0 : wa * axb);
          mm[0] = fmax(mm[0], fabs((axb - fmax(axb, 0.0)) / F[R_EA0 + k]));
          mm[2] += (last && wa != 0.0 && pya[k] > kVerifyTol) ? 1.0 : 0.0;
          mm[1] = fmax(mm[1], fabs((qa + u * py + bb * pya[k]) / F[R_DA0 + k]));
          ra[k] = -qa - u * e - bb * ea;
        }
        F[R_PY] = py;
        F[R_PYA0] = pya[0];
        F[R_PYA1] = pya[1];
        F[R_RA0] = ra[0];
        F[R_RA1] = ra[1];
        F[R_COEF] = last ? py : row_reduce_coef(F, ra[0], ra[1], -e);
      }
      __syncthreads();
      if (last) {
        scatter_columns<CNc>(q, [&](int i) { return q.v2[i] + q.qs[i] + q.beta[i] * q.yb[i]; });
      } else {
        scatter_columns<CNc>(q, [&](int i) {
          const double beta = q.beta[i];
          const double w = fabs(q.zb[i]);
          const double bnd = q.zb[i] > 0 ? q.ubs[i] : q.lbs[i];
          return -(q.v2[i] + q.qs[i]) - beta * (q.yb[i] + w * (beta * q.x[i] - bnd));
        });
      }
      for (int i = tid; i < N; i += kQpThreads) {
        const double beta = q.beta[i];
        const double ax = beta * q.x[i];
        const double w = fabs(q.zb[i]);
        const double lb = q.lbs[i], ub = q.ubs[i];
        const double zc = fmin(fmax(ax, lb), ub);
        mm[0] = fmax(mm[0], fabs((ax - zc) * q.Dz[i] / beta));
        const bool ineq = last && w != 0.0 && (ub - lb >= kRhoTol);
        mm[2] += (ineq && q.zb[i] > 0 && q.yb[i] < -kVerifyTol) ? 1.0 : 0.0;
        mm[2] += (ineq && q.zb[i] < 0 && q.yb[i] > kVerifyTol) ? 1.0 : 0.0;
        if (last) mm[1] = fmax(mm[1], fabs(q.v1[i] / q.Dz[i]));
      }
      if (last) {
        block_reduce<3, 0x4u>(q, mm);
        p_pri = mm[0];
        p_dua = mm[1] * q.cinv;
        verified = (mm[2] == 0.0) && (p_pri <= kVerifyTol) && isfinite(p_pri) && isfinite(p_dua);
      } else {
        bcr_solve<NB>(q, q.v1, q.w);
        for (int r = tid; r < q.nrows; r += kQpThreads) {
          const double* R = q.R(r);
          double* F = q.F(r);
          double a0, a1;
          row_backsub(F, row_dot<CNc>(q, R, q.I(r), q.w), a0, a1);
          F[R_PX0] += a0;
          F[R_PX1] += a1;
        }
        for (int i = tid; i < N; i += kQpThreads) {
          const double xn = q.x[i] + q.w[i];
          const double w = fabs(q.zb[i]);
          q.yb[i] += w * (q.beta[i] * xn - (q.zb[i] > 0 ? q.ubs[i] : q.lbs[i]));
          q.x[i] = xn;
        }
        __syncthreads();
      }
    }
    PROF_ADD(12);
#ifdef TB200_PROFILE
    if (tid == 0) atomicAdd(&g_prof[13], 1ull);
#endif
    return true;
  };
  auto restore_admm_state = [&](bool keep_polished_x) {
    for (int i = tid; i < q.Np; i += kQpThreads) {
      if (!keep_polished_x) q.x[i] = st_x[i];
      q.zb[i] = st_zb[i];
      q.yb[i] = st_yb[i];
    }
    __syncthreads();
  };

  bool done = !factor_ok;
  while (!done) {
    run_admm(polish_once, restore_admm_state);
    out.pri_res = pri_res;
    out.dua_res = dua_res;
    if (status != QPS_SOLVED || !st.polishing) {
      done = true;
    } else if (early_verified) {
      out.polish = 1;
      out.rounds = round;
      done = true;
    } else {
      bool verified = false;
      double p_pri = 0.0, p_dua = 0.0;
      if (use_pinv) stash_z(false);
      const bool factored = polish_once(verified, p_pri, p_dua);
      out.pol_factor_ok = factored ? 1 : 0;
      out.pol_pri = p_pri;
      out.pol_dua = p_dua;
      out.rounds = round;
      if (factored && verified) {
        out.polish = 1;
        done = true;
      } else if (round >= kVerifyRounds || iter >= st.max_iter) {
        const bool ok = factored && ((p_pri < pri_res && p_dua < dua_res) || (p_pri < pri_res && dua_res < 1e-10) ||
                                     (p_dua < dua_res && pri_res < 1e-10)) && isfinite(p_pri) && isfinite(p_dua);
        out.polish = ok ? 2 : -1;
        done = true;
      } else {
        ++round;
        eps_scale *= 0.1;
        restore_admm_state(false);
        if (use_pinv) {
          stash_z(true);
        } else if (!factorize(sysw)) {
          status = QPS_NONCVX;
          done = true;
        }
      }
    }
  }
  out.iters = iter;
  out.status = status;
  out.rho = rho;
  out.c = q.c;
  if (out.polish != 0) {
    if (out.polish > 0) {
      for (int r = tid; r < q.nrows; r += kQpThreads) {
        double* F = q.F(r);
        for (int k = 0; k < 2; ++k) F[R_XA0 + k] = F[R_PX0 + k];
      }
    }
    restore_admm_state(out.polish > 0);
  }
  return out;
}

template <int DD, int PAIR>
__device__ __noinline__ void qp_step(const DevProblem& p, const int b, const double* x_override ,
                                        const double* trust_override, int* admm_iters_out, int* polish_out) {
  constexpr int NB = 2 * DD;
  constexpr bool FG = DD > 8;
  extern __shared__ double sm[];
  const int tid = threadIdx.x;
  if (!x_override && (p.status[b] != 5 || p.qp_done[b] != 0)) return;
  const int N = p.N, T = p.T, D = p.D;
  QpCtx q;
  q.N = N; q.T = T; q.D = D; q.tid = tid;
  q.nb = NB;
  q.M = qp_block_count(N, NB);
  q.Np = q.M * NB;
  q.CN = (p.row_stride - R_NF) / 3;
  q.RS = p.row_stride;
  const QpSmem S = qp_smem_layout(N, NB, q.RS, q.CN, p.max_rows, FG);
  if (FG || !S.factor_smem) {
    double* fg = p.factor_g + static_cast<size_t>(blockIdx.x) * qp_cta_global_doubles(N, NB);
    const int fb = qp_even(q.M * NB * NB);
    q.SA = fg; q.SLM = fg + fb; q.SU = fg + 2 * fb;
  } else {
    q.SA = sm + S.SA; q.SLM = sm + S.SLM; q.SU = sm + S.SU;
  }
  q.beta = sm + S.beta;
  q.x = sm + S.x; q.zb = sm + S.zb; q.yb = sm + S.yb; q.v1 = sm + S.v1; q.w = sm + S.w;
  q.qs = sm + S.qs; q.lbs = sm + S.lbs; q.ubs = sm + S.ubs; q.tmp = sm + S.tmp; q.red = sm + S.red;
  q.flag = sm + S.red - 8;
  q.colptr = reinterpret_cast<int*>(sm + S.colptr);
  double* const rows_g = p.rows + static_cast<size_t>(b) * p.max_rows * p.row_stride;
  int* const rints_g = p.row_ints + static_cast<size_t>(b) * p.max_rows * RI_NINTS;
  q.rows = rows_g;
  q.soa = p.soa + static_cast<size_t>(blockIdx.x) * p.soa_stride;
  q.smbase = sm;
  q.pinv = S.pinv;
  q.pl = pinv_plan(q.M, NB);
  q.pi_g = p.factor_g + static_cast<size_t>(blockIdx.x) * qp_cta_global_doubles(N, NB);
  q.z_stash = q.pi_g + qp_factor_doubles(N, NB);
  q.rows_smem = 0;
  q.rints = rints_g;
  int* mylist = p.lists + static_cast<size_t>(b) * p.list_stride;
  int* colptr = mylist;
  int* colent = mylist + q.Np + 1;
  int* obj_start = colent + static_cast<size_t>(p.max_rows) * q.CN;
  q.colent = colent;
  q.band_offs = p.band_offs;
  q.n_band = p.n_band;
  if (S.pband_smem) {
    q.Pband = sm + S.Pb;
    for (int t = tid; t < N * (NB + 1); t += kQpThreads) sm[S.Pb + t] = p.Pband[t];
  } else {
    q.Pband = p.Pband;
  }
  double* gvec = p.scratch + static_cast<size_t>(b) * 5 * q.Np;
  q.scratch = gvec;
  q.Dz = sm + S.Dz;
  q.v2 = sm + S.v2;
  double *qs = q.qs, *lbs = q.lbs, *ubs = q.ubs;
  int* meta = p.ws_meta + static_cast<size_t>(b) * 8;
  const int n_obj = p.n_costs + p.n_cnts;
  int nr = 0, n_aux = 0, nnzA = 0;
  bool warm = false;
  int* sh_i = reinterpret_cast<int*>(q.flag + 2);

  {
    const double* xc = (x_override ? x_override : p.x) + static_cast<size_t>(b) * N;
    const double trust = trust_override ? trust_override[b] : p.trust[b];
    const double* mu = p.merit_coeffs + static_cast<size_t>(b) * p.n_cnts;
    const int buf = x_override ? 0 : p.cur_buf[b];
    const size_t slot = static_cast<size_t>(buf) * p.B + b;
    const double* cart_err = p.cart_err + slot * p.n_cart_rows;
    const double* cart_jac = p.cart_jac + slot * static_cast<size_t>(p.n_cart_rows) * p.cart_stride;
    const double* coll_rows = p.coll_rows + slot * static_cast<size_t>(p.n_coll_cand) * p.coll_stride;
    const unsigned long long* coll_mask = p.coll_mask + slot * static_cast<size_t>(p.n_coll_objs) * p.coll_words;

    for (int i = tid; i < N; i += kQpThreads) {
      const double lb = p.lower[i % D], ub = p.upper[i % D];
      const double xi = fmin(fmax(xc[i], lb), ub);
      lbs[i] = fmax(fmax(xi - trust, lb), -kOsqpInf);
      ubs[i] = fmin(fmin(xi + trust, ub), kOsqpInf);
      qs[i] = p.qlin[i];
      q.x[i] = xc[i];
    }
    __syncthreads();

    for (int f = tid; f < p.n_fixed; f += kQpThreads) {
      const int var = p.fixed_vars[f];
      double* R = q.R(f);
      int* I = q.rints + static_cast<size_t>(f) * RI_NINTS;
      for (int k = 0; k < q.CN; ++k) R[k] = (k == 0) ? 1.0 : 0.0;
      R[2 * q.CN + R_C] = -p.init_traj[static_cast<size_t>(b) * N + var];
      R[2 * q.CN + R_W] = 0.0;
      I[RI_BASE] = var; I[RI_CNT] = 1; I[RI_STRIDE] = D; I[RI_AUX] = AUX_NONE; I[RI_OBJ] = -1; I[RI_PAD] = 0;
    }
    nr += p.n_fixed;
    nnzA += p.n_fixed;
    int coll_obj_counter = 0;
    for (int oi = 0; oi < n_obj; ++oi) {
      const bool is_cnt = oi >= p.n_costs;
      const DevObj o = is_cnt ? p.cnt_objs[oi - p.n_costs] : p.cost_objs[oi];
      if (tid == 0) obj_start[oi] = nr;
      const double w_aux = is_cnt ? mu[oi - p.n_costs] : 1.0;
      if (o.kind == OBJ_JOINT_EQ_COST) continue;
      if (o.kind == OBJ_JOINT_EQ_CNT || o.kind == OBJ_JOINT_INEQ_CNT || o.kind == OBJ_JOINT_INEQ_COST) {
        const DevJointTerm& jt = p.joint_terms[o.term];
        const int per = (o.kind == OBJ_JOINT_EQ_CNT) ? 1 : 2;
        const int total = o.n_steps * D * per;
        const double wst[3][3] = {{1, 0, 0}, {-1, 1, 0}, {1, -2, 1}};
        for (int k = tid; k < total; k += kQpThreads) {
          const int t = o.first + k / (D * per), d = (k / per) % D, side = k % per;
          double* R = q.R(nr + k);
          int* I = q.rints + static_cast<size_t>(nr + k) * RI_NINTS;
          const double cd = jt.coeffs[d];
          double sgn = cd, cst;
          if (per == 1) cst = -jt.targets[d] * cd;
          else if (side == 0) cst = (-jt.targets[d] - jt.upper[d]) * cd;
          else { sgn = -cd; cst = (jt.lower[d] + jt.targets[d]) * cd; }
          for (int i = 0; i < q.CN; ++i) R[i] = (i <= o.order) ? wst[o.order][i] * sgn : 0.0;
          R[2 * q.CN + R_C] = cst;
          R[2 * q.CN + R_W] = w_aux;
          I[RI_BASE] = t * D + d; I[RI_CNT] = o.order + 1; I[RI_STRIDE] = D;
          I[RI_AUX] = (per == 1) ? AUX_ABS : AUX_HINGE; I[RI_OBJ] = oi;
          I[RI_PAD] = n_aux + k * ((per == 1) ? 2 : 1);
        }
        nr += total;
        n_aux += total * ((per == 1) ? 2 : 1);
        nnzA += total * (o.order + 1 + ((per == 1) ? 2 : 1));
      } else if (o.kind == OBJ_CART_POSE) {
        const DevCartTerm& ct = p.cart_terms[o.term];
        if (tid == 0) sh_i[0] = 0;
        __syncthreads();
        int nz = 0;
        for (int k = tid; k < o.n_rows; k += kQpThreads) {
          double* R = q.R(nr + k);
          int* I = q.rints + static_cast<size_t>(nr + k) * RI_NINTS;
          const double* J = cart_jac + static_cast<size_t>(o.src_off + k) * p.cart_stride;
          const double thr = 1e-7 * fabs(ct.coeff[k]);
          double dot = 0.0;
          for (int j = 0; j < q.CN; ++j) {
            const double Jj = (j < D) ? J[j] : 0.0;
            dot += Jj * q.x[o.first * D + min(j, D - 1)];
            const double a = (fabs(Jj) > thr) ? Jj : 0.0;
            R[j] = a;
            nz += (a != 0.0);
          }
          R[2 * q.CN + R_C] = cart_err[o.src_off + k] - dot;
          R[2 * q.CN + R_W] = w_aux;
          I[RI_BASE] = o.first * D; I[RI_CNT] = D; I[RI_STRIDE] = 1; I[RI_AUX] = AUX_ABS; I[RI_OBJ] = oi;
          I[RI_PAD] = n_aux + 2 * k;
        }
        if (nz) atomicAdd(&sh_i[0], nz);
        __syncthreads();
        nz = sh_i[0];
        __syncthreads();
        nr += o.n_rows;
        n_aux += 2 * o.n_rows;
        nnzA += nz + 2 * o.n_rows;
      } else if (o.kind == OBJ_CART_VEL) {
        if (tid == 0) sh_i[0] = 0;
        __syncthreads();
        int nz = 0;
        const int per = is_cnt ? 1 : 2;
        for (int k = tid; k < 6; k += kQpThreads) {
          double* R = q.R(nr + k);
          int* I = q.rints + static_cast<size_t>(nr + k) * RI_NINTS;
          const double* J = cart_jac + static_cast<size_t>(o.src_off + k) * p.cart_stride;
          double dot = 0.0;
          for (int j = 0; j < q.CN; ++j) {
            const double Jj = (j < 2 * D) ? J[j] : 0.0;
            dot += Jj * q.x[o.first * D + min(j, 2 * D - 1)];
            const double a = (fabs(Jj) > 1e-7) ? Jj : 0.0;
            R[j] = a;
            nz += (a != 0.0);
          }
          R[2 * q.CN + R_C] = cart_err[o.src_off + k] - dot;
          R[2 * q.CN + R_W] = w_aux;
          I[RI_BASE] = o.first * D; I[RI_CNT] = 2 * D; I[RI_STRIDE] = 1; I[RI_AUX] = is_cnt ? AUX_HINGE : AUX_ABS;
          I[RI_OBJ] = oi; I[RI_PAD] = n_aux + per * k;
        }
        if (nz) atomicAdd(&sh_i[0], nz);
        __syncthreads();
        nz = sh_i[0];
        __syncthreads();
        nr += 6;
        n_aux += per * 6;
        nnzA += nz + per * 6;
      } else if (o.kind == OBJ_COLL || o.kind == OBJ_COLL_CAST) {
        const unsigned long long* mw = coll_mask + static_cast<size_t>(coll_obj_counter) * p.coll_words;
        ++coll_obj_counter;
        if (tid == 0) { sh_i[0] = 0; sh_i[1] = 0; }
        __syncthreads();
        int nz = 0;
        for (int c = tid; c < o.n_rows; c += kQpThreads) {
          const bool act = (mw[c / 64] >> (c % 64)) & 1ull;
          if (act) {
            int before = 0;
            for (int wdx = 0; wdx < c / 64; ++wdx) before += __popcll(mw[wdx]);
            before += __popcll(mw[c / 64] & ((1ull << (c % 64)) - 1ull));
            const int pos = nr + before;
            double* R = q.R(pos);
            int* I = q.rints + static_cast<size_t>(pos) * RI_NINTS;
            const double* cr = coll_rows + static_cast<size_t>(o.src_off + c) * p.coll_stride;
            const int W = (o.kind == OBJ_COLL_CAST) ? 2 * D : D;
            const double thr = (o.kind == OBJ_COLL_CAST) ? 1e-7 : -1.0;
            const double scale = is_cnt ? cr[W + 2] : 1.0;
            double dot = 0.0;
            for (int j = 0; j < q.CN; ++j) {
              const double g = (j < W) ? cr[j] : 0.0;
              dot += g * q.x[o.first * D + min(j, W - 1)];
              const double a = (fabs(g) > thr) ? -g * scale : 0.0;
              R[j] = (j < W) ? a : 0.0;
              nz += (j < W && a != 0.0);
            }
            R[2 * q.CN + R_C] = (cr[W + 1] - cr[W] + dot) * scale;
            R[2 * q.CN + R_W] = is_cnt ? w_aux : cr[W + 2];
            I[RI_BASE] = o.first * D; I[RI_CNT] = W; I[RI_STRIDE] = 1; I[RI_AUX] = AUX_HINGE; I[RI_OBJ] = oi;
            I[RI_PAD] = n_aux + before;
          }
        }
        if (nz) atomicAdd(&sh_i[0], nz);
        __syncthreads();
        nz = sh_i[0];
        int count = 0;
        for (int wdx = 0; wdx < p.coll_words; ++wdx) count += __popcll(mw[wdx]);
        __syncthreads();
        nr += count;
        n_aux += count;
        nnzA += nz + count;
      }
    }
    if (tid == 0) obj_start[n_obj] = nr;
    nnzA += N + n_aux;
    __syncthreads();

    for (int i = tid; i <= q.Np; i += kQpThreads) colptr[i] = 0;
    __syncthreads();
    for (int r = tid; r < nr; r += kQpThreads) {
      const int* I = q.I(r);
      for (int k = 0; k < I[RI_CNT]; ++k) atomicAdd(&colptr[I[RI_BASE] + k * I[RI_STRIDE] + 1], 1);
    }
    __syncthreads();
    if (tid == 0)
      for (int i = 0; i < q.Np; ++i) colptr[i + 1] += colptr[i];
    __syncthreads();
    for (int i = tid; i < N; i += kQpThreads) {
      if (colptr[i + 1] == colptr[i]) continue;
      int pos = colptr[i];
      for (int r = 0; r < nr && pos < colptr[i + 1]; ++r) {
        const int* I = q.I(r);
        const int base = I[RI_BASE], stride = I[RI_STRIDE], cnt = I[RI_CNT];
        const int off = i - base;
        if (off >= 0 && off % stride == 0 && off / stride < cnt) colent[pos++] = (r << 5) | (off / stride);
      }
    }
    __syncthreads();
    q.nrows = nr;
  }
  for (int i = tid; i <= q.Np; i += kQpThreads) q.colptr[i] = colptr[i];
  __syncthreads();
  const bool rows_in_smem = nr <= S.row_cap;
  double* const rows_s = sm + S.rows;
  if (rows_in_smem) {
    int* rints_s = reinterpret_cast<int*>(sm + S.rints);
    int* colent_s = reinterpret_cast<int*>(sm + S.colent);
    for (int t = tid; t < nr * q.RS; t += kQpThreads) rows_s[t] = rows_g[t];
    for (int t = tid; t < nr * RI_NINTS; t += kQpThreads) rints_s[t] = rints_g[t];
    for (int t = tid; t < q.colptr[q.Np]; t += kQpThreads) colent_s[t] = colent[t];
    q.rows = rows_s;
    q.rows_smem = 1;
    q.rints = rints_s;
    q.colent = colent_s;
  }
  __syncthreads();

  warm = !x_override && p.qp.warm_starting && meta[3] == 1 && meta[0] == n_aux && meta[1] == nr && meta[2] == nnzA;
  { PROF_T0(); qp_scale(q, p.qp, n_aux); PROF_ADD(7); }
  __syncthreads();

  PROF_T0();
  QpOut res = qp_solve_block<NB, PAIR, (DD <= 7)>(q, p.qp, warm, p.ws_rho[b], p.ws_x + static_cast<size_t>(b) * N,
                                                  p.ws_yb + static_cast<size_t>(b) * N);
  __syncthreads();
  PROF_ADD(8);
#ifdef TB200_PROFILE
  if (tid == 0) atomicAdd(&g_prof[9], 1ull);
#endif

  double* nx = p.new_x + static_cast<size_t>(b) * N;
  for (int i = tid; i < N; i += kQpThreads) {
    const double xu = q.Dz[i] * q.x[i];
    nx[i] = xu;
    q.v1[i] = xu;
    p.ws_x[static_cast<size_t>(b) * N + i] = xu;
    p.ws_yb[static_cast<size_t>(b) * N + i] = q.cinv * (q.beta[i] / q.Dz[i]) * q.yb[i];
  }
  __syncthreads();
  for (int r = tid; r < nr; r += kQpThreads) {
    double* R = q.R(r);
    double* F = q.F(r);
    const int* I = q.I(r);
    const int aux = I[RI_AUX];
    F[R_Y] = q.cinv * F[R_E] * F[R_Y];
    for (int k = 0; k < 2; ++k) {
      F[R_XA0 + k] = (k < aux) ? F[R_DA0 + k] * F[R_XA0 + k] : 0.0;
      F[R_YA0 + k] = (k < aux) ? q.cinv * F[R_EA0 + k] * F[R_YA0 + k] : 0.0;
    }
    double val = F[R_C];
    for (int i = 0; i < I[RI_CNT]; ++i) val += R[i] * q.v1[I[RI_BASE] + i * I[RI_STRIDE]];
    F[R_MV] = (aux == AUX_ABS || aux == AUX_NONE) ? fabs(val) : fmax(val, 0.0);
  }
  __syncthreads();
  for (int oi = tid; oi < n_obj; oi += kQpThreads) {
    const bool is_cnt = oi >= p.n_costs;
    double s = 0.0;
    if (!is_cnt && p.cost_objs[oi].kind == OBJ_JOINT_EQ_COST) s = joint_obj_value(p, p.cost_objs[oi], q.v1);
    for (int r = obj_start[oi]; r < obj_start[oi + 1]; ++r) {
      const double* F = q.F(r);
      if (is_cnt) s += F[R_MV];
      else s += F[R_W] * (F[R_XA0] + F[R_XA1]);
    }
    if (is_cnt) p.model_cnt_viols[static_cast<size_t>(b) * p.n_cnts + (oi - p.n_costs)] = s;
    else p.model_cost_vals[static_cast<size_t>(b) * p.n_costs + oi] = s;
  }
  __syncthreads();
  if (rows_in_smem)
    for (int t = tid; t < nr * q.RS; t += kQpThreads) rows_g[t] = rows_s[t];
  if (tid == 0) {
    int cvx = 2;
    if (res.status == QPS_SOLVED || res.status == QPS_SOLVED_INACC) cvx = 0;
    else if (res.status >= QPS_PINF && res.status <= QPS_DINF_INACC) cvx = 1;
    p.qp_status[b] = cvx;
    meta[0] = n_aux; meta[1] = nr; meta[2] = nnzA; meta[3] = (cvx == 0) ? 1 : 0; meta[4] = 0;
    p.ws_rho[b] = res.rho;
    if (!x_override) {
      p.n_admm_iters[b] += res.iters;
      p.qp_done[b] = 1;
    }
    if (admm_iters_out) admm_iters_out[b] = res.iters;
    if (polish_out) polish_out[b] = res.polish;
    double* g = p.dbg + static_cast<size_t>(b) * 16;
    g[0] = res.status; g[1] = res.iters; g[2] = res.polish; g[3] = res.rho; g[4] = res.pri_res; g[5] = res.dua_res;
    g[6] = res.pol_pri; g[7] = res.pol_dua; g[8] = res.c; g[9] = res.pol_factor_ok; g[10] = res.rho_updates;
    g[11] = nr; g[12] = n_aux; g[13] = nnzA; g[14] = warm ? 1 : 0; g[15] = res.rounds;
  }
}

}
```

trajopt_b200/csrc/solve_inst.cuh:

```cuda
#include <cuda_runtime.h>

#include "solve_kernel.cuh"
#include "kernels.h"

#define TB200_CAT3_(a, b, c) a##b##_##c
#define TB200_CAT3(a, b, c) TB200_CAT3_(a, b, c)

namespace tb200 {
SolveKernelFn TB200_CAT3(solve_kernel_inst_, TB200_INST_D, TB200_INST_PAIR)() {
  return solve_kernel<TB200_INST_D, TB200_INST_PAIR>;
}
int TB200_CAT3(qp_prof_inst_, TB200_INST_D, TB200_INST_PAIR)(unsigned long long* out, int reset) {
#ifdef TB200_PROFILE
  if (reset) {
    unsigned long long z[16] = {0};
    cudaMemcpyToSymbol(g_prof, z, sizeof(z));
    return 0;
  }
  unsigned long long t[16];
  cudaMemcpyFromSymbol(t, g_prof, sizeof(t));
  for (int i = 0; i < 16; ++i) out[i] += t[i];
  return 0;
#else
  (void)out;
  (void)reset;
  return -1;
#endif
}
}
```

trajopt_b200/csrc/solve_kernels.cu:

```cuda
#include <cuda_runtime.h>

#include "kernels.h"

namespace tb200 {
#define TB200_INSTANCES(X) X(2, 0) X(3, 0) X(6, 0) X(7, 0) X(14, 0) X(2, 1) X(7, 1)
#define TB200_DECL(D, P)                  \
  SolveKernelFn solve_kernel_inst_##D##_##P(); \
  int qp_prof_inst_##D##_##P(unsigned long long*, int);
TB200_INSTANCES(TB200_DECL)
#undef TB200_DECL

SolveKernelFn solve_kernel_for(int D, bool pair_rows) {
#define TB200_PICK(DD, P) \
  if (D == DD && pair_rows == static_cast<bool>(P)) return solve_kernel_inst_##DD##_##P();
  TB200_INSTANCES(TB200_PICK)
#undef TB200_PICK
  return nullptr;
}
int qp_debug_prof(unsigned long long* out, int reset) {
  int rc = -1;
  if (!reset && out)
    for (int i = 0; i < 16; ++i) out[i] = 0;
#define TB200_PROF(D, P) \
  if (qp_prof_inst_##D##_##P(out, reset) == 0) rc = 0;
  TB200_INSTANCES(TB200_PROF)
#undef TB200_PROF
  return rc;
}
}
```

trajopt_b200/csrc/trajopt_b200.cu:

```cuda
#include <cuda_runtime.h>

#include <algorithm>
#include <cmath>
#include <cstdio>
#include <cstdlib>
#include <cstring>
#include <limits>
#include <memory>
#include <string>
#include <vector>

#include "../../include/trajopt_b200.h"
#include "eval_kernel.cuh"
#include "solve_kernel.cuh"
#include "kernels.h"

using namespace tb200;

namespace {
thread_local std::string g_err;
int fail(int code, const std::string& msg) {
  g_err = msg;
  return code;
}
// ... 335 lines not shown
      }
  P->cost_objs = costs;
  P->cnt_objs = eqs;
  P->cnt_objs.insert(P->cnt_objs.end(), ineqs.begin(), ineqs.end());
  const int n_eq = static_cast<int>(eqs.size());
  for (auto& r : cart_ref) {
    DevObj o = (r.first == 0) ? costs[r.second] : eqs[r.second];
    o.pad0 = r.second;
    P->cart_objs.push_back(o);
  }
  for (auto& r : vel_ref) {
    DevObj o = (r.first == 0) ? costs[r.second] : ineqs[r.second];
    o.pad0 = (r.first == 0) ? r.second : n_eq + r.second;
    P->vel_objs.push_back(o);
  }
  for (int pass = 0; pass < 2; ++pass)
    for (auto& r : coll_ref) {
      if ((pass == 0) != (r.first == 0)) continue;
      DevObj o = (r.first == 0) ? costs[r.second] : ineqs[r.second];
      o.pad0 = (r.first == 0) ? r.second : n_eq + r.second;
      P->coll_objs.push_back(o);
    }
  {
    int off = 0, k = 0;
    for (auto& o : P->coll_objs) {
      o.src_off = off;
      o.target_slot = k;
      off += o.n_rows;
      DevObj& m = o.is_cnt ? P->cnt_objs[o.pad0] : P->cost_objs[o.pad0];
      m.src_off = o.src_off;
      m.target_slot = k++;
    }
  }
  std::vector<int> fixed;
  for (int k = 0; k < d->n_fixed_timesteps; ++k) {
    const int t = d->fixed_timesteps[k];
    if (t < 0 || t >= T) return fail(TB200_ERR_INVALID, "Fixed timestep index is outside the bounds of the initial trajectory.");
    for (int j = 0; j < D; ++j) fixed.push_back(t * D + j);
  }
  for (int k = 0; k < d->n_fixed_dofs; ++k) {
    const int j = d->fixed_dofs[k];
    if (j < 0 || j >= D) return fail(TB200_ERR_INVALID, "DOF(aka Joint) indice is greater than the number of DOF available.");
    for (int t = 0; t < T; ++t) {
      bool skip = false;
      for (int f = 0; f < d->n_fixed_timesteps; ++f) skip |= d->fixed_timesteps[f] == t;
      if (!skip) fixed.push_back(t * D + j);
    }
  }
  max_rows += static_cast<int>(fixed.size());
  max_rows = std::max(max_rows, 1);

  const int W = dp.HB + 1;
  std::vector<double> Pband(static_cast<size_t>(N) * W, 0.0), qlin(N, 0.0);
  for (const DevObj& o : costs) {
    if (o.kind != OBJ_JOINT_EQ_COST) continue;
    static const double wst[3][3] = {{1, 0, 0}, {-1, 1, 0}, {1, -2, 1}};
    const DevJointTerm& jt = jts[o.term];
    for (int t = o.first; t < o.first + o.n_steps; ++t)
      for (int j = 0; j < D; ++j)
        for (int a = 0; a <= o.order; ++a) {
          const int ia = (t + a) * D + j;
          qlin[ia] += -2.0 * jt.coeffs[j] * jt.targets[j] * wst[o.order][a];
          for (int bb = 0; bb <= a; ++bb) {
            const int ib = (t + bb) * D + j;
            Pband[static_cast<size_t>(ia) * W + (ia - ib)] += 2.0 * jt.coeffs[j] * wst[o.order][a] * wst[o.order][bb];
          }
        }
  }

  {
    dp.n_band = 0;
    for (int k = 0; k < W; ++k) {
      bool nz = false;
      for (int i = k; i < N && !nz; ++i) nz = Pband[static_cast<size_t>(i) * W + k] != 0.0;
      if (nz) dp.band_offs[dp.n_band++] = k;
    }
  }
  dp.n_costs = static_cast<int>(P->cost_objs.size());
  dp.n_cnts = static_cast<int>(P->cnt_objs.size());
  dp.n_cart_rows = n_cart_rows;
  const int CN = (has_vel || has_cast) ? std::max(2 * D, 3) : std::max(D, 3);
  dp.cart_stride = has_vel ? 2 * D : D;
  dp.n_coll_cand = n_coll_cand;
  dp.coll_stride = has_cast ? 2 * D + 3 : D + 3;
  dp.n_fixed = static_cast<int>(fixed.size());
  dp.max_rows = max_rows;
  dp.row_stride = qp_row_stride(CN);
  dp.coll_words = std::max(1, ((has_cast ? cast_cap : dp.L * dp.O) + 63) / 64);
  dp.n_coll_objs = static_cast<int>(P->coll_objs.size());
  P->ex.n_cart_objs = static_cast<int>(P->cart_objs.size());
  P->ex.n_coll_objs = dp.n_coll_objs;
  P->ex.n_vel_objs = static_cast<int>(P->vel_objs.size());
  P->ex.cast = has_cast ? 1 : 0;
  P->ex.cast_cap = cast_cap;
  for (int sg = 0; sg < dp.S; ++sg)
    if (segs[sg].q_index >= 0) P->ex.joint_seg[segs[sg].q_index] = sg;
  P->ex.n_joint_objs = 0;
  {
    int idx = 0;
    auto note = [&](const DevObj& o) {
      if (o.kind <= OBJ_JOINT_INEQ_CNT) {
        if (P->ex.n_joint_objs < 8) P->ex.joint_obj_idx[P->ex.n_joint_objs] = idx;
        P->ex.n_joint_objs++;
      }
      ++idx;
    };
    for (const DevObj& o : P->cost_objs) note(o);
    for (const DevObj& o : P->cnt_objs) note(o);
    if (P->ex.n_joint_objs > 8) return fail(TB200_ERR_UNSUPPORTED, "more than 8 joint-space cost/constraint objects");
    if (dp.O > 64) return fail(TB200_ERR_UNSUPPORTED, "more than 64 obstacle spheres per trajectory");
  }
  P->layout.n_costs = dp.n_costs;
  P->layout.n_cnts = dp.n_cnts;
  P->layout.n_cart_rows = n_cart_rows;
  P->layout.cart_jac_stride = dp.cart_stride;
  P->layout.n_coll_cand = n_coll_cand;
  P->layout.coll_row_stride = dp.coll_stride;
  P->layout.n_vars = N;

  const EvalSmem es = eval_smem_layout(T, D, dp.L, dp.n_coll_objs, dp.n_coll_objs * dp.coll_words, dp.S, P->ex.n_joint_objs,
                                       P->ex.n_vel_objs, P->ex.cast, cast_cap, dp.n_costs + dp.n_cnts);
  P->pair_rows = (CN > std::max(D, 3));
  P->eval_smem = static_cast<size_t>(es.total) * sizeof(double);
  const bool factor_global = D > 8;
  const QpSmem qs = qp_smem_layout(N, 2 * D, dp.row_stride, CN, max_rows, factor_global);
  const int Np = qp_block_count(N, 2 * D) * 2 * D;
  dp.list_stride = static_cast<size_t>(Np + 1) + static_cast<size_t>(max_rows) * CN + dp.n_costs + dp.n_cnts + 2;
  P->qp_smem = static_cast<size_t>(qs.total) * sizeof(double);
  if (P->eval_smem > 226 * 1024 || P->qp_smem > 226 * 1024)
    return fail(TB200_ERR_UNSUPPORTED, "problem does not fit the 227 KB shared memory of one CTA");
  if (CN > 32) return fail(TB200_ERR_UNSUPPORTED, "more than 32 coefficients per QP row");
  if (!solve_kernel_for(D, P->pair_rows) || !eval_kernel_for(D))
    return fail(TB200_ERR_UNSUPPORTED, P->pair_rows ? "no kernel instance with two-waypoint rows (CartVel, continuous collision) for this number of joints"
                                                    : "no kernel instance for this number of joints");
  int ndev = 0;
  if (cudaGetDeviceCount(&ndev) != cudaSuccess || ndev == 0)
    return fail(TB200_ERR_NO_DEVICE, "no CUDA device: trajopt_b200 has no CPU fallback");
  if (device < 0 || device >= ndev) return fail(TB200_ERR_INVALID, "bad device ordinal");
  CK(cudaSetDevice(device));
  {
    size_t cur = 0;
    CK(cudaDeviceGetLimit(&cur, cudaLimitStackSize));
    if (cur < 6144) CK(cudaDeviceSetLimit(cudaLimitStackSize, 6144));
  }
  CK(cudaFuncSetAttribute(eval_kernel_for(D), cudaFuncAttributeMaxDynamicSharedMemorySize, static_cast<int>(P->eval_smem)));
  P->solve_smem = std::max(P->qp_smem, P->eval_smem);
  CK(cudaFuncSetAttribute(solve_kernel_for(D, P->pair_rows), cudaFuncAttributeMaxDynamicSharedMemorySize, static_cast<int>(P->solve_smem)));
  {
    int sms = 0;
    CK(cudaDeviceGetAttribute(&sms, cudaDevAttrMultiProcessorCount, device));
    P->n_sm = std::max(1, sms);
  }
  if (const char* e = std::getenv("TB200_QUANTUM")) P->quantum = std::max(1, std::atoi(e));
  CK(cudaStreamCreateWithFlags(&P->stream, cudaStreamNonBlocking));

#define ALLOC(buf, count) CK(P->buf.alloc(count))
#define UPLOAD(buf, vec) \
  CK(P->buf.alloc((vec).size())); \
  if (!(vec).empty()) CK(cudaMemcpy(P->buf.p, (vec).data(), (vec).size() * sizeof((vec)[0]), cudaMemcpyHostToDevice))
  UPLOAD(segs, segs);
  UPLOAD(spheres, sph);
  std::vector<double> lo(d->robot.lower, d->robot.lower + D), up(d->robot.upper, d->robot.upper + D);
  UPLOAD(lower, lo);
  UPLOAD(upper, up);
  UPLOAD(Pband, Pband);
  UPLOAD(qlin, qlin);
  UPLOAD(d_cost_objs, P->cost_objs);
  UPLOAD(d_cnt_objs, P->cnt_objs);
  UPLOAD(d_cart_objs, P->cart_objs);
  UPLOAD(d_coll_objs, P->coll_objs);
  UPLOAD(d_vel_objs, P->vel_objs);
  UPLOAD(joint_terms, jts);
  UPLOAD(cart_terms, cts);
  UPLOAD(fixed_vars, fixed);
  const size_t Bs = B;
  ALLOC(init_traj, Bs * N);
  ALLOC(cart_targets, Bs * std::max(1, d->n_cart_targets) * 7);
  ALLOC(obstacles, (d->obstacles_per_traj ? Bs : 1) * std::max(1, dp.O) * 4);
  ALLOC(x, Bs * N); ALLOC(new_x, Bs * N); ALLOC(trust, Bs); ALLOC(merit_coeffs, Bs * std::max(1, dp.n_cnts));
  ALLOC(cost_vals, Bs * std::max(1, dp.n_costs)); ALLOC(cnt_viols, Bs * std::max(1, dp.n_cnts));
  ALLOC(new_cost_vals, Bs * std::max(1, dp.n_costs)); ALLOC(new_cnt_viols, Bs * std::max(1, dp.n_cnts));
  ALLOC(model_cost_vals, Bs * std::max(1, dp.n_costs)); ALLOC(model_cnt_viols, Bs * std::max(1, dp.n_cnts));
  ALLOC(cart_err, 2 * Bs * std::max(1, n_cart_rows)); ALLOC(cart_jac, 2 * Bs * std::max(1, n_cart_rows) * dp.cart_stride);
  ALLOC(coll_rows, 2 * Bs * std::max(1, n_coll_cand) * dp.coll_stride);
  ALLOC(coll_mask, 2 * Bs * std::max(1, dp.n_coll_objs * dp.coll_words));
  ALLOC(rows, Bs * max_rows * dp.row_stride); ALLOC(row_ints, Bs * max_rows * RI_NINTS);
  ALLOC(lists, Bs * dp.list_stride);
  ALLOC(ws_x, Bs * N); ALLOC(ws_yb, Bs * N); ALLOC(scratch, Bs * 5 * Np); ALLOC(qp_done, Bs); ALLOC(ws_rho, Bs); ALLOC(ws_meta, Bs * 8);
  ALLOC(lvs_overflow, Bs);
  ALLOC(work_counter, 1);
  {
    int per_sm = 1;
    CK(cudaOccupancyMaxActiveBlocksPerMultiprocessor(&per_sm, eval_kernel_for(D), kEvalThreads, P->eval_smem));
    P->eval_grid = std::max(1, std::min(B, std::max(1, per_sm) * P->n_sm));
  }
  ALLOC(cast_scratch, has_cast ? static_cast<size_t>(std::max(P->eval_grid, std::min(B, P->n_sm))) * (kEvalThreads / 32) * 4 * cast_cap : 0);
  P->factor_grid = static_cast<size_t>(P->n_sm);
  ALLOC(factor_g, P->factor_grid * qp_cta_global_doubles(N, 2 * D));
  dp.soa_stride = (max_rows > qs.row_cap) ? qp_soa_doubles(max_rows, CN) : 0;
  ALLOC(soa, static_cast<size_t>(P->n_sm) * dp.soa_stride);
  {
    std::vector<int> chain(static_cast<size_t>(dp.S) * (kMaxSeg + 1), 0);
    for (int sg = 0; sg < dp.S; ++sg) {
      std::vector<int> up;
      for (int a = sg; a >= 0; a = segs[a].parent) up.push_back(a);
      int* c = chain.data() + static_cast<size_t>(sg) * (kMaxSeg + 1);
      c[0] = static_cast<int>(up.size());
      for (size_t k = 0; k < up.size(); ++k) c[1 + k] = up[up.size() - 1 - k];
    }
    UPLOAD(link_chain, chain);
  }
  ALLOC(status, Bs); ALLOC(sqp_iter, Bs); ALLOC(merit_round, Bs); ALLOC(qp_failures, Bs); ALLOC(qp_status, Bs);
  ALLOC(cur_buf, Bs); ALLOC(n_qp_solves, Bs); ALLOC(n_func_evals, Bs); ALLOC(n_admm_iters, Bs); ALLOC(active_count, 2);
  ALLOC(dbg, Bs * 16);
  ALLOC(sched_state, Bs); ALLOC(sched_timers, 8 + 2 * Bs);
  ALLOC(trace_len, Bs);
  ALLOC(x_tmp, Bs * N); ALLOC(trust_tmp, Bs); ALLOC(tmp_iters, Bs); ALLOC(tmp_polish, Bs);
#undef ALLOC
#undef UPLOAD
  dp.segs = P->segs.p; dp.spheres = P->spheres.p; dp.lower = P->lower.p; dp.upper = P->upper.p;
  dp.cost_objs = P->d_cost_objs.p; dp.cnt_objs = P->d_cnt_objs.p; dp.joint_terms = P->joint_terms.p;
  dp.cart_terms = P->cart_terms.p; dp.fixed_vars = P->fixed_vars.p; dp.Pband = P->Pband.p; dp.qlin = P->qlin.p;
  dp.init_traj = P->init_traj.p; dp.cart_targets = P->cart_targets.p; dp.obstacles = P->obstacles.p;
  dp.x = P->x.p; dp.new_x = P->new_x.p; dp.trust = P->trust.p; dp.merit_coeffs = P->merit_coeffs.p;
  dp.cost_vals = P->cost_vals.p; dp.cnt_viols = P->cnt_viols.p; dp.new_cost_vals = P->new_cost_vals.p;
  dp.new_cnt_viols = P->new_cnt_viols.p; dp.model_cost_vals = P->model_cost_vals.p; dp.model_cnt_viols = P->model_cnt_viols.p;
  dp.status = P->status.p; dp.sqp_iter = P->sqp_iter.p; dp.merit_round = P->merit_round.p; dp.qp_failures = P->qp_failures.p;
  dp.qp_status = P->qp_status.p; dp.cur_buf = P->cur_buf.p; dp.n_qp_solves = P->n_qp_solves.p;
  dp.n_func_evals = P->n_func_evals.p; dp.n_admm_iters = P->n_admm_iters.p; dp.active_count = P->active_count.p;
  dp.cart_err = P->cart_err.p; dp.cart_jac = P->cart_jac.p; dp.coll_rows = P->coll_rows.p; dp.coll_mask = P->coll_mask.p;
  dp.rows = P->rows.p; dp.row_ints = P->row_ints.p; dp.lists = P->lists.p; dp.ws_x = P->ws_x.p; dp.ws_yb = P->ws_yb.p;
  dp.scratch = P->scratch.p; dp.ws_meta = P->ws_meta.p; dp.ws_rho = P->ws_rho.p; dp.dbg = P->dbg.p; dp.sched_state = P->sched_state.p; dp.sched_timers = P->sched_timers.p; dp.trace_len = P->trace_len.p; dp.trace = nullptr; dp.trace_cap = 0;
  dp.soa = P->soa.p;
  dp.factor_g = P->factor_g.p; dp.lvs_overflow = P->lvs_overflow.p; dp.qp_done = P->qp_done.p;
  P->ex.link_chain = P->link_chain.p;
  P->ex.work_counter = P->work_counter.p;
  P->ex.cast_scratch = P->cast_scratch.p;
  P->ex.cart_objs = P->d_cart_objs.p;
  P->ex.coll_objs = P->d_coll_objs.p;
  P->ex.vel_objs = P->d_vel_objs.p;
  const tb200_qp_settings& q = d->qp;
  dp.qp = QpSettings{q.rho, q.sigma, q.alpha, q.eps_abs, q.eps_rel, q.eps_prim_inf, q.eps_dual_inf, q.delta,
                     q.adaptive_rho_tolerance, q.max_iter, q.scaling, q.check_termination, q.adaptive_rho,
                     q.adaptive_rho_interval, q.polishing, q.polish_refine_iter, q.warm_starting,
                     q.early_polish_every, q.early_polish_from};
  const tb200_sqp_params& s = d->sqp;
  dp.sqp = SqpParams{s.improve_ratio_threshold, s.min_trust_box_size, s.min_approx_improve, s.min_approx_improve_frac,
                     s.trust_shrink_ratio, s.trust_expand_ratio, s.cnt_tolerance, s.max_merit_coeff_increases,
                     s.merit_coeff_increase_ratio, s.initial_merit_error_coeff, s.trust_box_size, s.max_iter,
                     s.max_qp_solver_failures, s.inflate_constraints_individually, 0};
  int rc = tb200_problem_set_inputs(P, d->init_traj, d->cart_targets, d->obstacles);
  if (rc != TB200_OK) return rc;
  *out = guard.release();
  return TB200_OK;
}

void tb200_problem_destroy(tb200_problem* p) { delete p; }

int tb200_problem_layout(const tb200_problem* p, tb200_layout* out) {
  if (!p || !out) return fail(TB200_ERR_INVALID, "null argument");
  *out = p->layout;
  return TB200_OK;
}

int tb200_problem_set_sqp_params(tb200_problem* P, const tb200_sqp_params* s) {
  if (!P || !s) return fail(TB200_ERR_INVALID, "null argument");
  P->dp.sqp = SqpParams{s->improve_ratio_threshold, s->min_trust_box_size, s->min_approx_improve, s->min_approx_improve_frac,
                        s->trust_shrink_ratio, s->trust_expand_ratio, s->cnt_tolerance, s->max_merit_coeff_increases,
                        s->merit_coeff_increase_ratio, s->initial_merit_error_coeff, s->trust_box_size, s->max_iter,
                        s->max_qp_solver_failures, s->inflate_constraints_individually, 0};
  return TB200_OK;
}

int tb200_problem_set_inputs(tb200_problem* P, const double* init_traj, const double* cart_targets, const double* obstacles) {
  if (!P) return fail(TB200_ERR_INVALID, "null problem");
  CK(cudaSetDevice(P->device));
  P->timing.h2d_bytes = 0;
  if (init_traj) {
    CK(cudaMemcpyAsync(P->init_traj.p, init_traj, P->init_traj.n * sizeof(double), cudaMemcpyHostToDevice, P->stream));
    P->timing.h2d_bytes += static_cast<int64_t>(P->init_traj.n * sizeof(double));
  }
  if (cart_targets && P->dp.n_cart_targets > 0) {
    CK(cudaMemcpyAsync(P->cart_targets.p, cart_targets, P->cart_targets.n * sizeof(double), cudaMemcpyHostToDevice, P->stream));
    P->timing.h2d_bytes += static_cast<int64_t>(P->cart_targets.n * sizeof(double));
  }
  if (obstacles && P->dp.O > 0) {
    CK(cudaMemcpyAsync(P->obstacles.p, obstacles, P->obstacles.n * sizeof(double), cudaMemcpyHostToDevice, P->stream));
    P->timing.h2d_bytes += static_cast<int64_t>(P->obstacles.n * sizeof(double));
  }
  CK(cudaStreamSynchronize(P->stream));
  return TB200_OK;
}

namespace {
__global__ void reset_state_kernel(DevProblem p) {
  const int b = blockIdx.x * blockDim.x + threadIdx.x;
  if (b == 0) {
    p.active_count[0] = p.B;
    p.active_count[1] = 0;
    for (int k = 0; k < 8; ++k) p.sched_timers[k] = (k == 4) ? ~0ull : 0ull;
  }
  if (b >= p.B) return;
  p.status[b] = 5;
  p.sqp_iter[b] = 1;
  p.merit_round[b] = 0;
  p.qp_failures[b] = 0;
// ... 265 lines not shown
```

Before: 1338.

## Fuse QP residual checks and polish refinement into register-resident passes

Adds a fused convergence-check pass that computes the residual norms, infeasibility accumulators and an active-set hash inside the ADMM solve loop, using the per-thread register state already held there. Polish refinement moves into a dedicated noinline pass that computes row and variable updates together instead of calling separate generic matvec passes. Both paths are on by default and can be switched off with an environment variable. The aim is fewer shared-memory sweeps and barriers per check and per polish; the cost is extra register pressure and code size, plus a risk of small numerical differences from the generic path.

```diff
diff --git a/trajopt_b200/csrc/device_types.cuh b/trajopt_b200/csrc/device_types.cuh
--- a/trajopt_b200/csrc/device_types.cuh
+++ b/trajopt_b200/csrc/device_types.cuh
@@ -139,6 +139,7 @@
   int* sched_state;
   unsigned long long* sched_timers;
   QpSettings qp;
+  int qp_fast_passes;
   SqpParams sqp;
 };
 
diff --git a/trajopt_b200/csrc/kernels.h b/trajopt_b200/csrc/kernels.h
--- a/trajopt_b200/csrc/kernels.h
+++ b/trajopt_b200/csrc/kernels.h
@@ -9,5 +9,6 @@
 SolveKernelFn solve_kernel_for(int D, bool pair_rows);
 EvalKernelFn eval_kernel_for(int D);
 int eval_debug_prof(unsigned long long* out, int reset);
+constexpr int kQpProfSlots = 32;
 int qp_debug_prof(unsigned long long* out, int reset);
 }
diff --git a/trajopt_b200/csrc/qp_cta_kernel.cuh b/trajopt_b200/csrc/qp_cta_kernel.cuh
--- a/trajopt_b200/csrc/qp_cta_kernel.cuh
+++ b/trajopt_b200/csrc/qp_cta_kernel.cuh
@@ -5,12 +5,14 @@
 namespace tb200 {
 
 #ifdef TB200_PROFILE
-static __device__ unsigned long long g_prof[16];
+static __device__ unsigned long long g_prof[32];
 #define PROF_T0() const long long prof_t0_ = clock64()
 #define PROF_ADD(slot) do { if (q.tid == 0) atomicAdd(&g_prof[slot], (unsigned long long)(clock64() - prof_t0_)); } while (0)
+#define PROF_COUNT(slot) do { if (q.tid == 0) atomicAdd(&g_prof[slot], 1ull); } while (0)
 #else
 #define PROF_T0()
 #define PROF_ADD(slot)
+#define PROF_COUNT(slot)
 #endif
 #if defined(TB200_PROFILE) && defined(TB200_PROFILE_CHECK)
 #define PROF_CHK_T0() long long pc_ = clock64()
@@ -886,43 +888,145 @@
 }
 
 template <int NB>
+__device__ __forceinline__ double p_row(const QpCtx& q, const int i, const double* Dz, const double* vin) {
+  constexpr int HB = NB, W = HB + 1;
+  const int N = q.N, nbo = q.n_band;
+  const double* const Pb = q.Pband;
+  const int* const offs = q.band_offs;
+  double s = 0.0;
+  for (int t0 = 0; t0 < nbo; t0 += 4) {
+    double v[4];
+#pragma unroll
+    for (int u = 0; u < 4; ++u) {
+      const int k = (t0 + u < nbo) ? offs[t0 + u] : -1;
+      v[u] = (k >= 0 && k <= i) ? (Pb[i * W + k] * Dz[i - k]) * vin[i - k] : 0.0;
+    }
+    s += v[0]; s += v[1]; s += v[2]; s += v[3];
+  }
+  for (int t0 = 0; t0 < nbo; t0 += 4) {
+    double v[4];
+#pragma unroll
+    for (int u = 0; u < 4; ++u) {
+      const int k = (t0 + u < nbo) ? offs[t0 + u] : -1;
+      v[u] = (k >= 1 && i + k < N) ? (Pb[(i + k) * W + k] * Dz[i + k]) * vin[i + k] : 0.0;
+    }
+    s += v[0]; s += v[1]; s += v[2]; s += v[3];
+  }
+  return s * (q.c * Dz[i]);
+}
+template <int NB>
 __device__ __forceinline__ void p_matvec(const QpCtx& q, const double* in, double* out) {
   extern __shared__ double sm[];
-  constexpr int HB = NB, W = HB + 1;
-  const int N = q.N, Np = q.Np, nbo = q.n_band;
-  const double* const Pb = q.Pband;
+  const int N = q.N, Np = q.Np;
   const double* const Dz = sm + (q.Dz - q.smbase);
   const double* const vin = sm + (in - q.smbase);
   double* const vout = sm + (out - q.smbase);
-  const int* const offs = q.band_offs;
-  const double cc = q.c;
-  for (int i = q.tid; i < Np; i += kQpThreads) {
-    double s = 0.0;
-    if (i < N) {
-      for (int t0 = 0; t0 < nbo; t0 += 4) {
-        double v[4];
-#pragma unroll
-        for (int u = 0; u < 4; ++u) {
-          const int k = (t0 + u < nbo) ? offs[t0 + u] : -1;
-          v[u] = (k >= 0 && k <= i) ? (Pb[i * W + k] * Dz[i - k]) * vin[i - k] : 0.0;
-        }
-        s += v[0]; s += v[1]; s += v[2]; s += v[3];
-      }
-      for (int t0 = 0; t0 < nbo; t0 += 4) {
-        double v[4];
-#pragma unroll
-        for (int u = 0; u < 4; ++u) {
-          const int k = (t0 + u < nbo) ? offs[t0 + u] : -1;
-          v[u] = (k >= 1 && i + k < N) ? (Pb[(i + k) * W + k] * Dz[i + k]) * vin[i + k] : 0.0;
-        }
-        s += v[0]; s += v[1]; s += v[2]; s += v[3];
-      }
-      s *= cc * Dz[i];
-    }
-    vout[i] = s;
-  }
-  __syncthreads();
-}
+  for (int i = q.tid; i < Np; i += kQpThreads) vout[i] = (i < N) ? p_row<NB>(q, i, Dz, vin) : 0.0;
+  __syncthreads();
+}
+
+__device__ __forceinline__ void info_row_terms(const double* F, const double ax, double (&m)[14]) {
+  const double einv = 1.0 / F[R_E];
+  m[0] = fmax(m[0], fabs(einv * (ax - F[R_Z])));
+  m[1] = fmax(m[1], fabs(einv * F[R_Z]));
+  m[2] = fmax(m[2], fabs(einv * ax));
+  m[7] = fmax(m[7], fabs(ax - F[R_Z]));
+  m[8] = fmax(m[8], fabs(F[R_Z]));
+  m[9] = fmax(m[9], fabs(ax));
+#pragma unroll
+  for (int k = 0; k < 2; ++k) {
+    const double u = F[R_U0 + k], bb = F[R_B0 + k], qa = F[R_QA0 + k];
+    const double xa = F[R_XA0 + k], za = F[R_ZA0 + k], ya = F[R_YA0 + k];
+    const double iea = 1.0 / F[R_EA0 + k], ida = 1.0 / F[R_DA0 + k];
+    const double axb = bb * xa;
+    m[0] = fmax(m[0], fabs(iea * (axb - za)));
+    m[1] = fmax(m[1], fabs(iea * za));
+    m[2] = fmax(m[2], fabs(iea * axb));
+    m[7] = fmax(m[7], fabs(axb - za));
+    m[8] = fmax(m[8], fabs(za));
+    m[9] = fmax(m[9], fabs(axb));
+    const double aty = u * F[R_Y] + bb * ya;
+    m[3] = fmax(m[3], fabs(ida * (qa + aty)));
+    m[4] = fmax(m[4], fabs(ida * aty));
+    m[5] = fmax(m[5], fabs(ida * qa));
+    m[10] = fmax(m[10], fabs(qa + aty));
+    m[11] = fmax(m[11], fabs(aty));
+    m[12] = fmax(m[12], fabs(qa));
+  }
+}
+__device__ __forceinline__ void info_var_terms(const double dz, const double beta, const double x, const double zb,
+                                               const double aty, const double px, const double qv, double (&m)[14]) {
+  const double ax = beta * x;
+  const double einv = dz / beta, dinv = 1.0 / dz;
+  m[0] = fmax(m[0], fabs(einv * (ax - zb)));
+  m[1] = fmax(m[1], fabs(einv * zb));
+  m[2] = fmax(m[2], fabs(einv * ax));
+  m[7] = fmax(m[7], fabs(ax - zb));
+  m[8] = fmax(m[8], fabs(zb));
+  m[9] = fmax(m[9], fabs(ax));
+  const double d = qv + px + aty;
+  m[3] = fmax(m[3], fabs(dinv * d));
+  m[4] = fmax(m[4], fabs(dinv * aty));
+  m[5] = fmax(m[5], fabs(dinv * qv));
+  m[6] = fmax(m[6], fabs(dinv * px));
+  m[10] = fmax(m[10], fabs(d));
+  m[11] = fmax(m[11], fabs(aty));
+  m[12] = fmax(m[12], fabs(qv));
+  m[13] = fmax(m[13], fabs(px));
+}
+__device__ __forceinline__ double pinf_row_terms(const double* F, const int naux, double (&a)[3]) {
+  double d = F[R_DY];
+  d = (naux == AUX_HINGE) ? fmax(d, 0.0) : d;
+  a[0] = fmax(a[0], fabs(F[R_E] * d));
+  a[1] += F[R_UP] * fmax(d, 0.0) + F[R_LO] * fmin(d, 0.0);
+#pragma unroll
+  for (int k = 0; k < 2; ++k) {
+    const double da = fmin(F[R_DYA0 + k], 0.0);
+    a[0] = fmax(a[0], fabs(F[R_EA0 + k] * da));
+    a[2] = fmax(a[2], fabs((F[R_U0 + k] * d + F[R_B0 + k] * da) / F[R_DA0 + k]));
+  }
+  return d;
+}
+__device__ __forceinline__ void pinf_var_terms(const double ratio, const double ub, const double lb, const double d,
+                                               double (&a)[3]) {
+  a[0] = fmax(a[0], fabs(ratio * d));
+  a[1] += ub * fmax(d, 0.0) + lb * fmin(d, 0.0);
+}
+__device__ __forceinline__ void dinf_row_terms(const double* F, double (&a)[2]) {
+#pragma unroll
+  for (int k = 0; k < 2; ++k) {
+    a[0] = fmax(a[0], fabs(F[R_DA0 + k] * F[R_DXA0 + k]));
+    a[1] += F[R_QA0 + k] * F[R_DXA0 + k];
+  }
+}
+__device__ __forceinline__ unsigned long long guess_mix(unsigned long long v) {
+  v += 0x9e3779b97f4a7c15ull;
+  v = (v ^ (v >> 30)) * 0xbf58476d1ce4e5b9ull;
+  v = (v ^ (v >> 27)) * 0x94d049bb133111ebull;
+  return v ^ (v >> 31);
+}
+__device__ __forceinline__ unsigned long long guess_row_hash(const double* F, const int* I, const int r, const int nrows,
+                                                             const int N) {
+  unsigned long long h = 0ull;
+  const unsigned long long mc = static_cast<unsigned long long>(nrows);
+  if (F[R_Z] - F[R_LO] < -F[R_Y]) h += guess_mix(2ull * r);
+  else if (F[R_UP] - F[R_Z] < F[R_Y]) h += guess_mix(2ull * r + 1ull);
+  for (int k = 0; k < I[RI_AUX]; ++k) {
+    const unsigned long long idx = mc + N + I[RI_PAD] + k;
+    if (F[R_ZA0 + k] - 0.0 < -F[R_YA0 + k]) h += guess_mix(2ull * idx);
+    else if (kOsqpInf * F[R_EA0 + k] - F[R_ZA0 + k] < F[R_YA0 + k]) h += guess_mix(2ull * idx + 1ull);
+  }
+  return h;
+}
+__device__ __forceinline__ unsigned long long guess_var_hash(const double zb, const double yb, const double lb,
+                                                             const double ub, const int i, const int nrows) {
+  const unsigned long long idx = static_cast<unsigned long long>(nrows) + i;
+  if (zb - lb < -yb) return guess_mix(2ull * idx);
+  if (ub - zb < yb) return guess_mix(2ull * idx + 1ull);
+  return 0ull;
+}
+enum ChkQ { CHK_PA0 = 14, CHK_PA1, CHK_PA2, CHK_DA0, CHK_DA1, kChkHash };
+constexpr unsigned kChkSumMask = (1u << CHK_PA1) | (1u << CHK_DA1);
 
 __device__ inline void rows_prepare_weights(const QpCtx& q, const SysW& w) {
   for (int r = q.tid; r < q.nrows; r += kQpThreads) {
@@ -1558,6 +1662,9 @@
   constexpr int QN = 3 * NB;
   constexpr int kRowThreads = 64;
   extern __shared__ double sm[];
+#ifdef TB200_PROFILE
+  const long long prof_entry_ = clock64();
+#endif
   const int tid = q.tid, N = q.N, Np = q.Np, nrows = q.nrows, RS = q.RS;
   const double sigma = q.sigma, alpha = q.alpha, oma = 1.0 - q.alpha, rho = q.rho, rho_eq = q.rho_eq, rho_aux = rho_aux_in;
   const double inv_rho_aux = 1.0 / rho_aux, inv_rho = 1.0 / rho, inv_rho_eq = 1.0 / rho_eq;
@@ -1590,6 +1697,7 @@
   const bool v_eq = v_ub - v_lb < kRhoTol;
   const double v_rb = v_eq ? rho_eq : rho, v_irb = v_eq ? inv_rho_eq : inv_rho;
   double v_x = q.x[vi], v_z = q.zb[vi], v_y = q.yb[vi];
+  double v_dx = 0.0, v_dy = 0.0;
   const int e0 = has_var ? q.colptr[vi] : 0, e1 = has_var ? q.colptr[vi + 1] : 0;
   double* const zero_slot = sm + (q.flag - q.smbase) + 7;
   if (tid == 0) *zero_slot = 0.0;
@@ -1648,8 +1756,10 @@
       zn = fmin(fmax(zn, v_lb), v_ub);
       const double dy = v_rb * (zr - zn);
       if (keep_steps) {
-        dxs[vi] = xn - v_x;
-        dyb[vi] = dy;
+        v_dx = xn - v_x;
+        v_dy = dy;
+        dxs[vi] = v_dx;
+        dyb[vi] = v_dy;
       }
       v_x = xn;
       v_z = zn;
@@ -1662,6 +1772,9 @@
 #pragma unroll
     for (int j = 0; j < QN; ++j) pi[j] = prow ? q.pi_g[tid * QN + j] : 0.0;
     bar();
+#ifdef TB200_PROFILE
+    if (tid == 0) atomicAdd(&g_prof[21], (unsigned long long)(clock64() - prof_entry_));
+#endif
     for (int it = 0; it < n_iter; ++it) {
       const bool keep_steps = keep_last && it == n_iter - 1;
       { PROF_T0(); build_rhs(); PROF_ADD(1); }
@@ -1788,6 +1901,64 @@
     q.yb[vi] = v_y;
   }
   __syncthreads();
+  if (keep_last == 2) {
+    double m[14] = {0, 0, 0, 0, 0, 0, 0, 0, 0, 0, 0, 0, 0, 0};
+    double pa[3] = {0.0, 0.0, 0.0}, da[2] = {0.0, 0.0};
+    unsigned long long h = 0ull;
+    const double* const xs = sm + (q.x - q.smbase);
+    const double* const Dz = sm + (q.Dz - q.smbase);
+    if (has_var) {
+      const double px = p_row<NB>(q, vi, Dz, xs);
+      double aty = v_beta * v_y;
+      for (int e = e0; e < e1; ++e) {
+        const int ent = colent[e];
+        const double* R = rows + (ent >> 5) * RS;
+        aty += R[CNc + (ent & 31)] * R[2 * CNc + R_Y];
+      }
+      const double dz = Dz[vi];
+      info_var_terms(dz, v_beta, v_x, v_z, aty, px, v_qs, m);
+      pinf_var_terms(v_beta / dz, v_ub, v_lb, v_dy, pa);
+      da[0] = fmax(da[0], fabs(dz * v_dx));
+      da[1] += v_qs * v_dx;
+      h += guess_var_hash(v_z, v_y, v_lb, v_ub, vi, nrows);
+    }
+    if (upper) {
+      for (int r = kQpThreads - 1 - tid; r < nrows; r += kRowThreads) {
+        const double* R = rows + r * RS;
+        double* F = rows + r * RS + 2 * CNc;
+        const int* I = rints + r * RI_NINTS;
+        const double ax = row_dot<CNc>(q, R, I, xs) + F[R_U0] * F[R_XA0] + F[R_U1] * F[R_XA1];
+        info_row_terms(F, ax, m);
+        pinf_row_terms(F, I[RI_AUX], pa);
+        dinf_row_terms(F, da);
+        h += guess_row_hash(F, I, r, nrows, N);
+      }
+    }
+    double vals[kChkHash] = {m[0], m[1], m[2], m[3], m[4], m[5], m[6], m[7], m[8], m[9], m[10], m[11], m[12], m[13],
+                             pa[0], pa[1], pa[2], da[0], da[1]};
+    static_assert(CHK_PA0 == 14 && CHK_DA1 == 18, "vals[] follows ChkQ");
+    __syncwarp();
+#pragma unroll
+    for (int k = 0; k < kChkHash; ++k) {
+      double v = vals[k];
+      if ((kChkSumMask >> k) & 1u) {
+#pragma unroll
+        for (int off = 16; off > 0; off >>= 1) v += __shfl_xor_sync(0xffffffffu, v, off);
+      } else {
+        v = warp_max_norm(v);
+      }
+      vals[k] = v;
+    }
+    for (int off = 16; off > 0; off >>= 1) h += __shfl_xor_sync(0xffffffffu, h, off);
+    if ((tid & 31) == 0) {
+      double* const chk = sm + (q.tmp - q.smbase);
+      const int wid = tid >> 5;
+#pragma unroll
+      for (int k = 0; k < kChkHash; ++k) chk[k * 8 + wid] = vals[k];
+      reinterpret_cast<unsigned long long*>(chk + kChkHash * 8)[wid] = h;
+    }
+    __syncthreads();
+  }
 }
 
 enum SoaF { S_U0 = 0, S_U1, S_B0, S_B1, S_LO, S_UP, S_QA0, S_QA1, S_WRR, S_IWRR, S_G0, S_G1, S_IDEN, S_UPA0, S_UPA1,
@@ -2078,9 +2249,121 @@
   __syncthreads();
 }
 
+struct PolishRes {
+  double p_pri, p_dua, bad;
+};
+template <int NB, int PAIR>
+__device__ __noinline__ PolishRes polish_passes(const QpCtx& q, const int refine_iter) {
+  constexpr int CNc = PAIR ? ((NB > 3) ? NB : 3) : ((NB / 2 > 3) ? NB / 2 : 3);
+  constexpr int kRowThreads = 64;
+  extern __shared__ double sm[];
+  const int tid = q.tid, N = q.N, Np = q.Np, nrows = q.nrows, RS = q.RS;
+  double* const rows = sm + (q.rows - q.smbase);
+  const int* const rints = reinterpret_cast<const int*>(sm + (reinterpret_cast<const double*>(q.rints) - q.smbase));
+  const int* const colent = reinterpret_cast<const int*>(sm + (reinterpret_cast<const double*>(q.colent) - q.smbase));
+  double* const xs = sm + (q.x - q.smbase);
+  double* const v1 = sm + (q.v1 - q.smbase);
+  double* const w = sm + (q.w - q.smbase);
+  const double* const Dz = sm + (q.Dz - q.smbase);
+  const SolveRoles roles = solve_roles<NB>(q);
+  const bool upper = tid >= kQpThreads - kRowThreads;
+  const bool has_var = tid < N;
+  const int vi = has_var ? tid : 0;
+  const double v_beta = q.beta[vi], v_lb = q.lbs[vi], v_ub = q.ubs[vi], v_qs = q.qs[vi], v_dz = Dz[vi], v_zb = q.zb[vi];
+  const double v_w = fabs(v_zb), v_bnd = v_zb > 0 ? v_ub : v_lb;
+  const int e0 = has_var ? q.colptr[vi] : 0, e1 = has_var ? q.colptr[vi + 1] : 0;
+  double v_x = q.x[vi], v_y = q.yb[vi];
+  const double cinv = q.cinv;
+  __syncthreads();
+  for (int it = 0; it <= refine_iter + 1; ++it) {
+    const bool last = (it == refine_iter + 1);
+    double mm[3] = {0.0, 0.0, 0.0};
+    double px = 0.0;
+    if (has_var) px = p_row<NB>(q, vi, Dz, xs);
+    if (upper) {
+      for (int r = kQpThreads - 1 - tid; r < nrows; r += kRowThreads) {
+        const double* R = rows + r * RS;
+        double* F = rows + r * RS + 2 * CNc;
+        const int* I = rints + r * RI_NINTS;
+        const int naux = I[RI_AUX];
+        const double Wr = F[R_WRR];
+        const double ax = row_dot<CNc>(q, R, I, xs) + F[R_U0] * F[R_PX0] + F[R_U1] * F[R_PX1];
+        const double py = F[R_PY] + ((it > 0) ? Wr * (ax - F[R_PB]) : 0.0);
+        const double e = py + (last ? 0.0 : Wr * (ax - F[R_PB]));
+        const double zc = fmin(fmax(ax, F[R_LO]), F[R_UP]);
+        mm[0] = fmax(mm[0], fabs((ax - zc) / F[R_E]));
+        mm[2] += (last && Wr != 0.0 && naux == AUX_HINGE && py < -kVerifyTol) ? 1.0 : 0.0;
+        double pya[2], ra[2];
+#pragma unroll
+        for (int k = 0; k < 2; ++k) {
+          const double bb = F[R_B0 + k], u = F[R_U0 + k], qa = F[R_QA0 + k];
+          const double wa = fabs(F[R_PWA0 + k]);
+          const double axb = bb * F[R_PX0 + k];
+          pya[k] = F[R_PYA0 + k] + ((it > 0) ? wa * axb : 0.0);
+          const double ea = pya[k] + (last ? 0.0 : wa * axb);
+          mm[0] = fmax(mm[0], fabs((axb - fmax(axb, 0.0)) / F[R_EA0 + k]));
+          mm[2] += (last && wa != 0.0 && pya[k] > kVerifyTol) ? 1.0 : 0.0;
+          mm[1] = fmax(mm[1], fabs((qa + u * py + bb * pya[k]) / F[R_DA0 + k]));
+          ra[k] = -qa - u * e - bb * ea;
+        }
+        F[R_PY] = py;
+        F[R_PYA0] = pya[0];
+        F[R_PYA1] = pya[1];
+        F[R_RA0] = ra[0];
+        F[R_RA1] = ra[1];
+        F[R_COEF] = last ? py : row_reduce_coef(F, ra[0], ra[1], -e);
+      }
+    }
+    __syncthreads();
+    if (tid < Np) {
+      double s = 0.0;
+      if (has_var) {
+        s = last ? px + v_qs + v_beta * v_y : -(px + v_qs) - v_beta * (v_y + v_w * (v_beta * v_x - v_bnd));
+        for (int e = e0; e < e1; ++e) {
+          const int ent = colent[e];
+          const double* R = rows + (ent >> 5) * RS;
+          s += R[CNc + (ent & 31)] * R[2 * CNc + R_COEF];
+        }
+        const double ax = v_beta * v_x;
+        const double zc = fmin(fmax(ax, v_lb), v_ub);
+        mm[0] = fmax(mm[0], fabs((ax - zc) * v_dz / v_beta));
+        const bool ineq = last && v_w != 0.0 && (v_ub - v_lb >= kRhoTol);
+        mm[2] += (ineq && v_zb > 0 && v_y < -kVerifyTol) ? 1.0 : 0.0;
+        mm[2] += (ineq && v_zb < 0 && v_y > kVerifyTol) ? 1.0 : 0.0;
+        if (last) mm[1] = fmax(mm[1], fabs(s / v_dz));
+      }
+      v1[tid] = s;
+    }
+    if (last) {
+      if (has_var) q.yb[vi] = v_y;
+      block_reduce<3, 0x4u>(q, mm);
+      return PolishRes{mm[0], mm[1] * cinv, mm[2]};
+    }
+    bcr_solve_sm<NB>(tid, roles, sm, v1, w);
+    if (upper) {
+      for (int r = kQpThreads - 1 - tid; r < nrows; r += kRowThreads) {
+        const double* R = rows + r * RS;
+        double* F = rows + r * RS + 2 * CNc;
+        double a0, a1;
+        row_backsub(F, row_dot<CNc>(q, R, rints + r * RI_NINTS, w), a0, a1);
+        F[R_PX0] += a0;
+        F[R_PX1] += a1;
+      }
+    }
+    if (has_var) {
+      const double xn = v_x + w[vi];
+      v_y += v_w * (v_beta * xn - v_bnd);
+      v_x = xn;
+      xs[vi] = xn;
+    }
+    __syncthreads();
+  }
+  return PolishRes{0.0, 0.0, 0.0};
+}
+
 template <int NB, int PAIR, bool REGOK>
 __device__ inline QpOut qp_solve_block(QpCtx& q, const QpSettings& st, bool warm, double warm_rho,
-                                       const double* ws_x, const double* ws_yb) {
+                                       const double* ws_x, const double* ws_yb, const bool fast_passes) {
   constexpr int CNc = PAIR ? ((NB > 3) ? NB : 3) : ((NB / 2 > 3) ? NB / 2 : 3);
   const int N = q.N, tid = q.tid;
   QpOut out{QPS_UNSOLVED, 0, 0, st.rho, 0, 0, 0, 0, 0, -1, 0, 0};
@@ -2136,12 +2419,16 @@
   const bool use_reg = REGOK && solve_roles_fit(q.M, NB);
   const bool use_pinv = REGOK && q.pinv && q.rows_smem;
   using BlockFn = void (*)(const QpCtx&, double, int, int);
+  const bool fuse = use_pinv && fast_passes;
+  const bool fast_polish = use_pinv && fast_passes && q.Np <= kQpThreads && solve_roles_fit(q.M, NB);
+  bool fused_chk = false;
   auto run_block = [&](int n, bool keep_last) {
+    fused_chk = fuse && keep_last;
     if constexpr (REGOK) {
       if (use_pinv || use_reg) {
         BlockFn volatile fn = use_pinv ? &admm_block_pinv<NB, PAIR>
                                        : (q.rows_smem ? &admm_block_fast<NB, PAIR> : &admm_block_soa<NB, PAIR>);
-        fn(q, sysw.rho_aux, n, keep_last ? 1 : 0);
+        fn(q, sysw.rho_aux, n, keep_last ? (fuse ? 2 : 1) : 0);
         return;
       }
     }
@@ -2150,6 +2437,7 @@
   };
   using FactorFn = bool (*)(const QpCtx&, const SysW&);
   auto factorize = [&](const SysW& wts) -> bool {
+    fused_chk = false;
     if constexpr (REGOK) {
       if (use_pinv && !wts.polish) {
         FactorFn volatile fn = &assemble_factor<NB, true>;
@@ -2192,58 +2480,14 @@
       const double* R = q.R(r);
       double* F = q.F(r);
       const double ax = row_dot<CNc>(q, R, q.I(r), q.x) + F[R_U0] * F[R_XA0] + F[R_U1] * F[R_XA1];
-      const double einv = 1.0 / F[R_E];
-      m[0] = fmax(m[0], fabs(einv * (ax - F[R_Z])));
-      m[1] = fmax(m[1], fabs(einv * F[R_Z]));
-      m[2] = fmax(m[2], fabs(einv * ax));
-      m[7] = fmax(m[7], fabs(ax - F[R_Z]));
-      m[8] = fmax(m[8], fabs(F[R_Z]));
-      m[9] = fmax(m[9], fabs(ax));
-#pragma unroll
-      for (int k = 0; k < 2; ++k) {
-        const double u = F[R_U0 + k], bb = F[R_B0 + k], qa = F[R_QA0 + k];
-        const double xa = F[R_XA0 + k], za = F[R_ZA0 + k], ya = F[R_YA0 + k];
-        const double iea = 1.0 / F[R_EA0 + k], ida = 1.0 / F[R_DA0 + k];
-        const double axb = bb * xa;
-        m[0] = fmax(m[0], fabs(iea * (axb - za)));
-        m[1] = fmax(m[1], fabs(iea * za));
-        m[2] = fmax(m[2], fabs(iea * axb));
-        m[7] = fmax(m[7], fabs(axb - za));
-        m[8] = fmax(m[8], fabs(za));
-        m[9] = fmax(m[9], fabs(axb));
-        const double aty = u * F[R_Y] + bb * ya;
-        m[3] = fmax(m[3], fabs(ida * (qa + aty)));
-        m[4] = fmax(m[4], fabs(ida * aty));
-        m[5] = fmax(m[5], fabs(ida * qa));
-        m[10] = fmax(m[10], fabs(qa + aty));
-        m[11] = fmax(m[11], fabs(aty));
-        m[12] = fmax(m[12], fabs(qa));
-      }
+      info_row_terms(F, ax, m);
       F[R_COEF] = F[R_Y];
     }
     __syncthreads();
     PROF_CHK(14);
     scatter_columns<CNc>(q, [&](int i) { return q.beta[i] * q.yb[i]; });
-    for (int i = tid; i < N; i += kQpThreads) {
-      const double dz = q.Dz[i], beta = q.beta[i];
-      const double ax = beta * q.x[i], aty = q.v1[i], px = q.v2[i];
-      const double einv = dz / beta, dinv = 1.0 / dz;
-      m[0] = fmax(m[0], fabs(einv * (ax - q.zb[i])));
-      m[1] = fmax(m[1], fabs(einv * q.zb[i]));
-      m[2] = fmax(m[2], fabs(einv * ax));
-      m[7] = fmax(m[7], fabs(ax - q.zb[i]));
-      m[8] = fmax(m[8], fabs(q.zb[i]));
-      m[9] = fmax(m[9], fabs(ax));
-      const double qv = q.qs[i], d = qv + px + aty;
-      m[3] = fmax(m[3], fabs(dinv * d));
-      m[4] = fmax(m[4], fabs(dinv * aty));
-      m[5] = fmax(m[5], fabs(dinv * qv));
-      m[6] = fmax(m[6], fabs(dinv * px));
-      m[10] = fmax(m[10], fabs(d));
-      m[11] = fmax(m[11], fabs(aty));
-      m[12] = fmax(m[12], fabs(qv));
-      m[13] = fmax(m[13], fabs(px));
-    }
+    for (int i = tid; i < N; i += kQpThreads)
+      info_var_terms(q.Dz[i], q.beta[i], q.x[i], q.zb[i], q.v1[i], q.v2[i], q.qs[i], m);
     if (scaled) {
       block_reduce<14, 0u>(q, m);
       s_pri = m[7]; s_z = m[8]; s_ax = m[9]; s_dua = m[10]; s_aty = m[11]; s_q = m[12]; s_px = m[13];
@@ -2259,30 +2503,51 @@
     n_z = m[1]; n_ax = m[2]; n_aty = m[4]; n_q = m[5]; n_px = m[6];
   };
 
+  auto fused_q = [&](const int k) -> double {
+    extern __shared__ double sm[];
+    const double* const chk = sm + (q.tmp - q.smbase) + k * 8;
+    if ((kChkSumMask >> k) & 1u) {
+      double acc = chk[0];
+      for (int w = 1; w < kQpThreads / 32; ++w) acc += chk[w];
+      return acc;
+    }
+    return warp_max_norm(chk[tid & 7]);
+  };
+  auto residuals = [&](const bool scaled) {
+    if (!fused_chk) {
+      info_pass(scaled);
+      return;
+    }
+    double m[14];
+#pragma unroll
+    for (int k = 0; k < 14; ++k) m[k] = (k < 7 || scaled) ? fused_q(k) : 0.0;
+    pri_res = m[0];
+    dua_res = m[3] * q.cinv;
+    n_z = m[1]; n_ax = m[2]; n_aty = m[4]; n_q = m[5]; n_px = m[6];
+    if (scaled) { s_pri = m[7]; s_z = m[8]; s_ax = m[9]; s_dua = m[10]; s_aty = m[11]; s_q = m[12]; s_px = m[13]; }
+  };
+
   auto primal_infeasible = [&](double eps) -> bool {
     double a[3] = {0.0, 0.0, 0.0};
-    for (int r = tid; r < q.nrows; r += kQpThreads) {
-      double* F = q.F(r);
-      const int naux = q.I(r)[RI_AUX];
-      double d = F[R_DY];
-      d = (naux == AUX_HINGE) ? fmax(d, 0.0) : d;
-      a[0] = fmax(a[0], fabs(F[R_E] * d));
-      a[1] += F[R_UP] * fmax(d, 0.0) + F[R_LO] * fmin(d, 0.0);
-      F[R_COEF] = d;
-#pragma unroll
-      for (int k = 0; k < 2; ++k) {
-        const double da = fmin(F[R_DYA0 + k], 0.0);
-        a[0] = fmax(a[0], fabs(F[R_EA0 + k] * da));
-        a[2] = fmax(a[2], fabs((F[R_U0 + k] * d + F[R_B0 + k] * da) / F[R_DA0 + k]));
-      }
-    }
-    for (int i = tid; i < N; i += kQpThreads) {
-      const double d = dyb[i];
-      a[0] = fmax(a[0], fabs(q.beta[i] / q.Dz[i] * d));
-      a[1] += q.ubs[i] * fmax(d, 0.0) + q.lbs[i] * fmin(d, 0.0);
-    }
-    block_reduce<3, 0x2u>(q, a);
+    if (fused_chk) {
+      a[0] = fused_q(CHK_PA0); a[1] = fused_q(CHK_PA1); a[2] = fused_q(CHK_PA2);
+    } else {
+      for (int r = tid; r < q.nrows; r += kQpThreads) {
+        double* F = q.F(r);
+        F[R_COEF] = pinf_row_terms(F, q.I(r)[RI_AUX], a);
+      }
+      for (int i = tid; i < N; i += kQpThreads) pinf_var_terms(q.beta[i] / q.Dz[i], q.ubs[i], q.lbs[i], dyb[i], a);
+      block_reduce<3, 0x2u>(q, a);
+    }
     if (!((a[0] > eps) && (a[1] < -eps * a[0]))) return false;
+    if (fused_chk) {
+      double unused[3] = {0.0, 0.0, 0.0};
+      for (int r = tid; r < q.nrows; r += kQpThreads) {
+        double* F = q.F(r);
+        F[R_COEF] = pinf_row_terms(F, q.I(r)[RI_AUX], unused);
+      }
+      __syncthreads();
+    }
     scatter_columns<CNc>(q, [&](int i) { return q.beta[i] * dyb[i]; });
     double mm[1] = {a[2]};
     for (int i = tid; i < N; i += kQpThreads) mm[0] = fmax(mm[0], fabs(q.v1[i] / q.Dz[i]));
@@ -2291,25 +2556,20 @@
   };
   auto dual_infeasible = [&](double eps) -> bool {
     double a[2] = {0.0, 0.0};
-    for (int i = tid; i < q.Np; i += kQpThreads) {
-      const double dxi = (i < N) ? dxs[i] : 0.0;
-      if (i < N) {
-        a[0] = fmax(a[0], fabs(q.Dz[i] * dxi));
-        a[1] += q.qs[i] * dxi;
-      }
-      q.v1[i] = dxi;
-    }
-    for (int r = tid; r < q.nrows; r += kQpThreads) {
-      const double* F = q.F(r);
-#pragma unroll
-      for (int k = 0; k < 2; ++k) {
-        a[0] = fmax(a[0], fabs(F[R_DA0 + k] * F[R_DXA0 + k]));
-        a[1] += F[R_QA0 + k] * F[R_DXA0 + k];
-      }
-    }
-    block_reduce<2, 0x2u>(q, a);
+    if (fused_chk) {
+      a[0] = fused_q(CHK_DA0); a[1] = fused_q(CHK_DA1);
+    } else {
+      for (int i = tid; i < N; i += kQpThreads) {
+        a[0] = fmax(a[0], fabs(q.Dz[i] * dxs[i]));
+        a[1] += q.qs[i] * dxs[i];
+      }
+      for (int r = tid; r < q.nrows; r += kQpThreads) dinf_row_terms(q.F(r), a);
+      block_reduce<2, 0x2u>(q, a);
+    }
     const double ndx = a[0], qdx = a[1];
     if (!((ndx > eps) && (qdx < -q.c * eps * ndx))) return false;
+    for (int i = tid; i < q.Np; i += kQpThreads) q.v1[i] = (i < N) ? dxs[i] : 0.0;
+    __syncthreads();
     p_matvec<NB>(q, q.v1, q.v2);
     double b2[2] = {0.0, 0.0};
     for (int i = tid; i < N; i += kQpThreads) {
@@ -2354,39 +2614,24 @@
     return res;
   };
 
-  auto guess_mix = [](unsigned long long v) -> unsigned long long {
-    v += 0x9e3779b97f4a7c15ull;
-    v = (v ^ (v >> 30)) * 0xbf58476d1ce4e5b9ull;
-    v = (v ^ (v >> 27)) * 0x94d049bb133111ebull;
-    return v ^ (v >> 31);
-  };
   auto early_guess_settled = [&]() -> bool {
     unsigned long long h = 0ull;
-    const unsigned long long mc = static_cast<unsigned long long>(q.nrows);
-    for (int r = tid; r < q.nrows; r += kQpThreads) {
-      const double* F = q.F(r);
-      const int* I = q.I(r);
-      if (F[R_Z] - F[R_LO] < -F[R_Y]) h += guess_mix(2ull * r);
-      else if (F[R_UP] - F[R_Z] < F[R_Y]) h += guess_mix(2ull * r + 1ull);
-      for (int k = 0; k < I[RI_AUX]; ++k) {
-        const unsigned long long idx = mc + N + I[RI_PAD] + k;
-        if (F[R_ZA0 + k] - 0.0 < -F[R_YA0 + k]) h += guess_mix(2ull * idx);
-        else if (kOsqpInf * F[R_EA0 + k] - F[R_ZA0 + k] < F[R_YA0 + k]) h += guess_mix(2ull * idx + 1ull);
-      }
-    }
-    for (int i = tid; i < N; i += kQpThreads) {
-      const unsigned long long idx = mc + i;
-      if (q.zb[i] - q.lbs[i] < -q.yb[i]) h += guess_mix(2ull * idx);
-      else if (q.ubs[i] - q.zb[i] < q.yb[i]) h += guess_mix(2ull * idx + 1ull);
-    }
-    __syncwarp();
-    for (int off = 16; off > 0; off >>= 1) h += __shfl_xor_sync(0xffffffffu, h, off);
-    unsigned long long* red = reinterpret_cast<unsigned long long*>(q.red.ptr());
-    if ((tid & 31) == 0) red[tid >> 5] = h;
-    __syncthreads();
-    h = 0ull;
-    for (int w = 0; w < kQpThreads / 32; ++w) h += red[w];
-    __syncthreads();
+    if (fused_chk) {
+      extern __shared__ double sm[];
+      const unsigned long long* hw = reinterpret_cast<const unsigned long long*>(sm + (q.tmp - q.smbase) + kChkHash * 8);
+      for (int w = 0; w < kQpThreads / 32; ++w) h += hw[w];
+    } else {
+      for (int r = tid; r < q.nrows; r += kQpThreads) h += guess_row_hash(q.F(r), q.I(r), r, q.nrows, N);
+      for (int i = tid; i < N; i += kQpThreads) h += guess_var_hash(q.zb[i], q.yb[i], q.lbs[i], q.ubs[i], i, q.nrows);
+      __syncwarp();
+      for (int off = 16; off > 0; off >>= 1) h += __shfl_xor_sync(0xffffffffu, h, off);
+      unsigned long long* red = reinterpret_cast<unsigned long long*>(q.red.ptr());
+      if ((tid & 31) == 0) red[tid >> 5] = h;
+      __syncthreads();
+      h = 0ull;
+      for (int w = 0; w < kQpThreads / 32; ++w) h += red[w];
+      __syncthreads();
+    }
     const bool stable = have_prev_guess && h == prev_guess;
     prev_guess = h;
     have_prev_guess = true;
@@ -2399,7 +2644,7 @@
     bool stop = false;
     while (!stop) {
       if (iter >= st.max_iter) {
-        if (!(st.check_termination > 0 && (iter % st.check_termination == 0))) info_pass(false);
+        if (!(st.check_termination > 0 && (iter % st.check_termination == 0))) residuals(false);
         status = check_termination(true);
         if (status == QPS_UNSOLVED) status = QPS_MAXITER;
         stop = true;
@@ -2413,17 +2658,24 @@
         run_block(n, can_check || iter == st.max_iter);
         if (can_check) {
           PROF_T0();
-          info_pass(rho_iter);
+          residuals(rho_iter);
           PROF_CHK_T0();
           status = check_termination(false);
           PROF_CHK(9);
           PROF_ADD(5);
+          bool try_early = false;
           if (status != QPS_UNSOLVED) stop = true;
           else if (st.polishing && st.early_polish_every > 0 && iter >= st.early_polish_from &&
-                   (iter % st.early_polish_every == 0) && early_guess_settled()) {
+                   (iter % st.early_polish_every == 0)) {
+            PROF_T0();
+            try_early = early_guess_settled();
+            PROF_ADD(22);
+          }
+          if (try_early) {
             bool verified = false;
             double p_pri = 0.0, p_dua = 0.0;
-            if (use_pinv) stash_z(false);
+            PROF_COUNT(17);
+            { PROF_T0(); if (use_pinv) stash_z(false); PROF_ADD(16); }
             const bool factored = polish_fn(verified, p_pri, p_dua);
             if (factored && verified) {
               early_verified = true;
@@ -2433,21 +2685,22 @@
               status = QPS_SOLVED;
               stop = true;
             } else {
+              PROF_T0();
               failed_guess = pending_guess;
               have_failed_guess = true;
               restore_fn(false);
-              info_pass(rho_iter);
               if (use_pinv) {
                 stash_z(true);
               } else if (!factorize(sysw)) {
                 status = QPS_NONCVX;
                 stop = true;
               }
+              PROF_ADD(19);
             }
           }
         }
         if (!stop && rho_iter) {
-          if (!can_check) info_pass(true);
+          if (!can_check) residuals(true);
           const double pn = s_pri / (fmax(s_z, s_ax) + 1e-10);
           const double dn = s_dua / (fmax(s_q, fmax(s_aty, s_px)) + 1e-10);
           double rho_new = rho * sqrt(pn / (dn + 1e-10));
@@ -2458,10 +2711,12 @@
             q.rho_eq = kRhoEqOverIneq * rho;
             sysw.rho_aux = rho;
             out.rho_updates++;
+            PROF_T0();
             if (!factorize(sysw)) {
               status = QPS_NONCVX;
               stop = true;
             }
+            PROF_ADD(20);
           }
         }
       }
@@ -2470,46 +2725,20 @@
 
   const double wp = 1.0 / st.delta;
   const SysW pw{true, st.delta, 0.0};
-  auto polish_once = [&](bool& verified, double& p_pri, double& p_dua) -> bool {
+  auto polish_refine = [&](bool& verified, double& p_pri, double& p_dua) {
     PROF_T0();
-    verified = false;
-    for (int i = tid; i < q.Np; i += kQpThreads) {
-      const double z = q.zb[i], y = q.yb[i];
-      double w = 0.0;
-      if (i < N) {
-        if (z - q.lbs[i] < -y) w = -wp;
-        else if (q.ubs[i] - z < y) w = wp;
-      }
-      st_x[i] = q.x[i];
-      st_zb[i] = z;
-      st_yb[i] = y;
-      q.zb[i] = w;
-      q.x[i] = 0.0;
-      q.yb[i] = 0.0;
-    }
-    for (int r = tid; r < q.nrows; r += kQpThreads) {
-      double* F = q.F(r);
-      const int naux = q.I(r)[RI_AUX];
-      double w = 0.0, b = 0.0;
-      if (F[R_Z] - F[R_LO] < -F[R_Y]) { w = -wp; b = F[R_LO]; }
-      else if (F[R_UP] - F[R_Z] < F[R_Y]) { w = wp; b = F[R_UP]; }
-      F[R_PW] = w;
-      F[R_PB] = b;
-      F[R_PY] = 0.0;
-#pragma unroll
-      for (int k = 0; k < 2; ++k) {
-        double wa = 0.0;
-        if (k < naux) {
-          if (F[R_ZA0 + k] - 0.0 < -F[R_YA0 + k]) wa = -wp;
-          else if (kOsqpInf * F[R_EA0 + k] - F[R_ZA0 + k] < F[R_YA0 + k]) wa = wp;
-        }
-        F[R_PWA0 + k] = wa;
-        F[R_PYA0 + k] = 0.0;
-        F[R_PX0 + k] = 0.0;
-      }
-    }
-    __syncthreads();
-    if (!factorize(pw)) return false;
+    if constexpr (REGOK) {
+      if (fast_polish) {
+        using PassFn = PolishRes (*)(const QpCtx&, int);
+        PassFn volatile fn = &polish_passes<NB, PAIR>;
+        const PolishRes res = fn(q, st.polish_refine_iter);
+        p_pri = res.p_pri;
+        p_dua = res.p_dua;
+        verified = (res.bad == 0.0) && (p_pri <= kVerifyTol) && isfinite(p_pri) && isfinite(p_dua);
+        PROF_ADD(12);
+        return;
+      }
+    }
     for (int it = 0; it <= st.polish_refine_iter + 1; ++it) {
       const bool last = (it == st.polish_refine_iter + 1);
       p_matvec<NB>(q, q.x, q.v2);
@@ -2593,9 +2822,52 @@
       }
     }
     PROF_ADD(12);
-#ifdef TB200_PROFILE
-    if (tid == 0) atomicAdd(&g_prof[13], 1ull);
-#endif
+  };
+  auto polish_once = [&](bool& verified, double& p_pri, double& p_dua) -> bool {
+    PROF_COUNT(13);
+    PROF_T0();
+    verified = false;
+    for (int i = tid; i < q.Np; i += kQpThreads) {
+      const double z = q.zb[i], y = q.yb[i];
+      double w = 0.0;
+      if (i < N) {
+        if (z - q.lbs[i] < -y) w = -wp;
+        else if (q.ubs[i] - z < y) w = wp;
+      }
+      st_x[i] = q.x[i];
+      st_zb[i] = z;
+      st_yb[i] = y;
+      q.zb[i] = w;
+      q.x[i] = 0.0;
+      q.yb[i] = 0.0;
+    }
+    for (int r = tid; r < q.nrows; r += kQpThreads) {
+      double* F = q.F(r);
+      const int naux = q.I(r)[RI_AUX];
+      double w = 0.0, b = 0.0;
+      if (F[R_Z] - F[R_LO] < -F[R_Y]) { w = -wp; b = F[R_LO]; }
+      else if (F[R_UP] - F[R_Z] < F[R_Y]) { w = wp; b = F[R_UP]; }
+      F[R_PW] = w;
+      F[R_PB] = b;
+      F[R_PY] = 0.0;
+#pragma unroll
+      for (int k = 0; k < 2; ++k) {
+        double wa = 0.0;
+        if (k < naux) {
+          if (F[R_ZA0 + k] - 0.0 < -F[R_YA0 + k]) wa = -wp;
+          else if (kOsqpInf * F[R_EA0 + k] - F[R_ZA0 + k] < F[R_YA0 + k]) wa = wp;
+        }
+        F[R_PWA0 + k] = wa;
+        F[R_PYA0 + k] = 0.0;
+        F[R_PX0 + k] = 0.0;
+      }
+    }
+    __syncthreads();
+    PROF_ADD(16);
+    bool factored;
+    { PROF_T0(); factored = factorize(pw); PROF_ADD(23); }
+    if (!factored) return false;
+    polish_refine(verified, p_pri, p_dua);
     return true;
   };
   auto restore_admm_state = [&](bool keep_polished_x) {
@@ -2621,7 +2893,8 @@
     } else {
       bool verified = false;
       double p_pri = 0.0, p_dua = 0.0;
-      if (use_pinv) stash_z(false);
+      PROF_COUNT(18);
+      { PROF_T0(); if (use_pinv) stash_z(false); PROF_ADD(16); }
       const bool factored = polish_once(verified, p_pri, p_dua);
       out.pol_factor_ok = factored ? 1 : 0;
       out.pol_pri = p_pri;
@@ -2638,6 +2911,7 @@
       } else {
         ++round;
         eps_scale *= 0.1;
+        PROF_T0();
         restore_admm_state(false);
         if (use_pinv) {
           stash_z(true);
@@ -2645,6 +2919,7 @@
           status = QPS_NONCVX;
           done = true;
         }
+        PROF_ADD(19);
       }
     }
   }
@@ -2944,7 +3219,7 @@
 
   PROF_T0();
   QpOut res = qp_solve_block<NB, PAIR, (DD <= 7)>(q, p.qp, warm, p.ws_rho[b], p.ws_x + static_cast<size_t>(b) * N,
-                                                  p.ws_yb + static_cast<size_t>(b) * N);
+                                                  p.ws_yb + static_cast<size_t>(b) * N, p.qp_fast_passes != 0);
   __syncthreads();
   PROF_ADD(8);
 #ifdef TB200_PROFILE
diff --git a/trajopt_b200/csrc/solve_inst.cuh b/trajopt_b200/csrc/solve_inst.cuh
--- a/trajopt_b200/csrc/solve_inst.cuh
+++ b/trajopt_b200/csrc/solve_inst.cuh
@@ -12,14 +12,15 @@
 }
 int TB200_CAT3(qp_prof_inst_, TB200_INST_D, TB200_INST_PAIR)(unsigned long long* out, int reset) {
 #ifdef TB200_PROFILE
+  static_assert(sizeof(g_prof) == kQpProfSlots * sizeof(unsigned long long), "g_prof and kQpProfSlots disagree");
   if (reset) {
-    unsigned long long z[16] = {0};
+    unsigned long long z[kQpProfSlots] = {0};
     cudaMemcpyToSymbol(g_prof, z, sizeof(z));
     return 0;
   }
-  unsigned long long t[16];
+  unsigned long long t[kQpProfSlots];
   cudaMemcpyFromSymbol(t, g_prof, sizeof(t));
-  for (int i = 0; i < 16; ++i) out[i] += t[i];
+  for (int i = 0; i < kQpProfSlots; ++i) out[i] += t[i];
   return 0;
 #else
   (void)out;
diff --git a/trajopt_b200/csrc/solve_kernels.cu b/trajopt_b200/csrc/solve_kernels.cu
--- a/trajopt_b200/csrc/solve_kernels.cu
+++ b/trajopt_b200/csrc/solve_kernels.cu
@@ -20,7 +20,7 @@
 int qp_debug_prof(unsigned long long* out, int reset) {
   int rc = -1;
   if (!reset && out)
-    for (int i = 0; i < 16; ++i) out[i] = 0;
+    for (int i = 0; i < kQpProfSlots; ++i) out[i] = 0;
 #define TB200_PROF(D, P) \
   if (qp_prof_inst_##D##_##P(out, reset) == 0) rc = 0;
   TB200_INSTANCES(TB200_PROF)
diff --git a/trajopt_b200/csrc/trajopt_b200.cu b/trajopt_b200/csrc/trajopt_b200.cu
--- a/trajopt_b200/csrc/trajopt_b200.cu
+++ b/trajopt_b200/csrc/trajopt_b200.cu
@@ -511,6 +511,10 @@
     P->n_sm = std::max(1, sms);
   }
   if (const char* e = std::getenv("TB200_QUANTUM")) P->quantum = std::max(1, std::atoi(e));
+  {
+    const char* e = std::getenv("TB200_GENERIC_QP_PASSES");
+    P->dp.qp_fast_passes = (e && std::atoi(e) != 0) ? 0 : 1;
+  }
   CK(cudaStreamCreateWithFlags(&P->stream, cudaStreamNonBlocking));
 
 #define ALLOC(buf, count) CK(P->buf.alloc(count))
```

Result: faster. 1405, median of 6 (+5.0%).
